# ChuckDanz/DCLIP

Measured on AMD Instinct MI355X. Metric: distill-step images/sec at ViT-B/32 bs=256, higher is better.
Workload: dtype f32

## Files before the change

dclip_amd/_lib.py:

```python
from __future__ import annotations

import ctypes as C
import os

_HERE = os.path.dirname(os.path.abspath(__file__))
LIB_PATH = os.environ.get("DCLIP_LIB_PATH") or os.path.join(_HERE, "libdclip_hip.so")

P = C.c_void_p
I = C.c_int
F = C.c_float
Z = C.c_size_t
L = C.c_int64

SIGNATURES = {
    "dclip_abi_version": (I, []),
    "dclip_last_error": (C.c_char_p, []),
    "dclip_last_launch": (C.c_char_p, []),
    "dclip_first_launch": (C.c_char_p, []),
    "dclip_gemm_f32_workspace": (Z, [I, I, I, I, I]),
    "dclip_gemm_f32_plan": (I, [I, I, I, I, I, C.POINTER(C.c_int)]),
    "dclip_gemm_f32": (I, [P, P, P, P, P, P, I, I, I, I, I, I, I, I, F, I, P, Z, P]),
    "dclip_colsum_f32_workspace": (Z, [I, I]),
    "dclip_colsum_f32": (I, [P, P, I, I, I, I, P, Z, P]),
    "dclip_layernorm_fwd": (I, [P, P, P, P, P, P, I, I, F, P]),
# ... 85 lines not shown
    "dclip_adamw_f32": (I, [P, P, P, P, Z, F, F, F, F, F, I, P, P]),
    "dclip_mt_record_bytes": (I, []),
    "dclip_mt_chunk_elems": (I, []),
    "dclip_mt_sumsq_f32": (I, [P, I, I, P, P]),
    "dclip_mt_adamw_f32": (I, [P, I, I, F, F, F, F, F, P, P]),
    "dclip_mt_adam_f32": (I, [P, I, I, F, F, F, F, F, P, P]),
    "dclip_axpby": (I, [P, P, F, F, Z, P]),
    "dclip_fill": (I, [P, F, Z, P]),
    "dclip_gemm_f16": (I, [P, P, P, P, P, I, I, I, I, I, I, I, I, P]),
    "dclip_cast_f32_f16": (I, [P, P, I, I, I, I, P]),
    "dclip_layernorm_fwd_f16": (I, [P, P, P, P, I, I, F, P]),
    "dclip_im2col_f16": (I, [P, P, I, I, I, I, I, I, P]),
    "dclip_attention_fwd_f16": (I, [P, P, I, I, I, I, P]),
    "dclip_attention_row_fwd_f16": (I, [P, P, P, I, I, I, P]),
    "dclip_split_f32_f16x3": (I, [P, P, I, I, I, I, F, I, P]),
    "dclip_layernorm_fwd_f16x3": (I, [P, P, P, P, I, I, F, F, P]),
    "dclip_gemm_f16_scaled": (I, [P, P, P, P, P, I, I, I, I, I, I, I, I, F, P]),
    "dclip_gemm_f16_scaled_split": (I, [P, P, P, P, I, I, I, I, I, I, I, F, F, P]),
    "dclip_split_f32_f16x3_dev": (I, [P, P, I, I, I, I, P, I, P]),
    "dclip_layernorm_fwd_f16x3_dev": (I, [P, P, P, P, P, P, P, I, I, F, P, P]),
    "dclip_gemm_f16_scaled_dev": (I, [P, P, P, P, P, I, I, I, I, I, I, I, I, P, P]),
    "dclip_gemm_f16_scaled_split_dev": (I, [P, P, P, P, P, P, I, I, I, I, I, I, I, P, P, P]),
    "dclip_split16_record_bytes": (I, []),
    "dclip_split16_plan_floats": (I, []),
    "dclip_split16_tile_rows": (I, []),
    "dclip_split16_stats": (I, [P, I, I, P, P]),
    "dclip_split16_plan": (I, [P, P, I, I, P]),
    "dclip_split16_weights": (I, [P, I, I, P, P]),
    "dclip_split_f32_f16x3_rows": (I, [P, P, P, I, I, I, P]),
    "dclip_split16_weights_t": (I, [P, I, I, P, P, P]),
    "dclip_gemm_f16_scaled_rows_dev": (I, [P, P, P, P, I, I, I, I, I, I, I, P, P, P]),
    "dclip_split_f32_f16x3_rows_colstats_workspace": (Z, [I, I]),
    "dclip_split_f32_f16x3_rows_colstats": (I, [P, P, P, P, P, P, P, I, I, I, P, Z, P]),
    "dclip_gemm_f16_wgrad_tokmajor_seg3_plan": (I, [I, I, I]),
    "dclip_gemm_f16_wgrad_tokmajor_seg3": (I, [P, P, P, I, I, I, I, I, I, I, I, I, I, I, I, P, P, I, P, Z, P]),
    "dclip_gemm_f16_ex": (I, [P, P, P, P, P, P, I, I, I, I, I, I, I, I, P]),
    "dclip_gemm_f16_wgrad_tokmajor_plan": (I, [I, I, I]),
    "dclip_gemm_f16_wgrad_tokmajor": (I, [P, P, P, I, I, I, I, I, I, I, P, Z, P]),
    "dclip_gemm_f16_splitk_plan": (I, [I, I, I]),
    "dclip_gemm_f16_splitk_workspace": (Z, [I, I, I]),
    "dclip_gemm_f16_splitk": (I, [P, P, P, I, I, I, I, I, I, I, P, Z, P]),
    "dclip_cast_f32_f16_ieee": (I, [P, P, I, I, I, I, P]),
    "dclip_layernorm_fwd_f16_stats": (I, [P, P, P, P, P, P, I, I, F, P]),
    "dclip_layernorm_bwd_ex_f16": (I, [P, P, P, P, P, P, P, P, P, P, P, I, I, I, P, Z, P]),
    "dclip_transpose_to_f16": (I, [P, I, P, P, I, I, I, I, I, P]),
    "dclip_rowsum_f16": (I, [P, P, I, I, I, P]),
    "dclip_colsum_f16": (I, [P, P, I, I, I, I, P, Z, P]),
    "dclip_mt_weights_f16": (I, [P, I, I, P]),
    "dclip_attention_fwd_f16_lse": (I, [P, P, P, I, I, I, I, P]),
    "dclip_attention_bwd_f16": (I, [P, P, P, P, P, I, I, I, I, P]),
    "dclip_clip_coef_scaled": (I, [P, I, F, P, P, P]),
    "dclip_mt_adamw_f32_skip": (I, [P, I, I, F, F, F, F, F, P, P]),
    "dclip_amp_update_scale": (I, [P, P, P, F, F, I, P]),
}

_lib = None


class DclipError(RuntimeError):
    pass


def load():
    global _lib
    if _lib is not None:
        return _lib
# ... 20 lines not shown
```

dclip_amd/csrc/attention.hip:

```cpp
#include "common.h"
#include "attention_tiles.h"
#include <stdlib.h>

namespace {

typedef unsigned short u16x4a __attribute__((ext_vector_type(4)));
typedef unsigned short u16x8a __attribute__((ext_vector_type(8)));
__device__ __forceinline__ f32x4 bf4_to_f32(u16x4a b) {
  f32x4 v;
#pragma unroll
  for (int e = 0; e < 4; ++e) v[e] = __builtin_bit_cast(float, (unsigned int)b[e] << 16);
  return v;
}
__device__ __forceinline__ u16x4a f32_to_bf4(f32x4 v) {
  u16x4a b;
#pragma unroll
  for (int e = 0; e < 4; ++e) b[e] = __builtin_bit_cast(unsigned short, (__bf16)v[e]);
  return b;
}
__device__ __forceinline__ void commit8(float* tile, int row, int chunk, u16x8a b, bool zero) {
  f32x4 lo, hi;
#pragma unroll
  for (int e = 0; e < 4; ++e) {
    lo[e] = zero ? 0.f : __builtin_bit_cast(float, (unsigned int)b[e] << 16);
// ... 511 lines not shown
    zero4(dpt);
    mma_rows_x_tileT(st, kf, t0, lane);
    mma_rows_x_tileT(dpt, vf, t1, lane);
#pragma unroll
    for (int nt = 0; nt < 4; ++nt) {
      const int ql = nt * 16 + l15, q = q0 + ql;
      const float lq = lse_s[ql], dq_ = dl_s[ql];
#pragma unroll
      for (int r = 0; r < 4; ++r) {
        const int key = k0 + 16 * wave + 4 * qd + r;
        const bool masked = key >= S || q >= Sq || (CAUSAL && key > q);
        const float p = masked ? 0.f : __expf(st[nt][r] * kScale - lq);
        scp[(4 * qd + r) * SCR + ql] = p;
        scs[(4 * qd + r) * SCR + ql] = p * (dpt[nt][r] - dq_) * kScale;
      }
    }
    __syncthreads();
    mma_scratch_x_tile(dv, scp, t1, lane);
    mma_scratch_x_tile(dk, scs, t0, lane);
  }
#pragma unroll
  for (int r = 0; r < 4; ++r) {
    const int key = k0 + 16 * wave + 4 * qd + r;
    if (key < S)
#pragma unroll
      for (int nt = 0; nt < 4; ++nt) {
        const size_t o = ((size_t)b * S + key) * lddkv + h * HD + nt * 16 + l15;
        dk_out[o] = dk[nt][r];
        dv_out[o] = dv[nt][r];
      }
  }
}

template <bool CAUSAL, bool IO16 = false>
__global__ void __launch_bounds__(256, 3) attn_bwd_lean_kernel(AttnArgs a, const float* __restrict__ out,
                                                               const float* __restrict__ dout, const float* __restrict__ lse,
                                                               float* __restrict__ dq_out, float* __restrict__ dk_out,
                                                               float* __restrict__ dv_out, int ldd) {
  __shared__ __attribute__((aligned(16))) float lds[3 * TS * HD + 2 * TS];
  float* Qs = lds;
  float* dOs = lds + TS * HD;
  float* dSs = lds + 2 * TS * HD;
  float* lse_s = lds + 3 * TS * HD;
  float* dl_s = lse_s + TS;
  const int H = a.H, S = a.Sk;
  const int lane = threadIdx.x & 63, wave = threadIdx.x >> 6;
  const int qd = lane >> 4, l15 = lane & 15;
  const int bh = blockIdx.x, b = bh / H, h = bh % H;
  const int D = H * HD;
  const int own = 16 * wave + l15, ownc = min(own, S - 1);
  const float my_lse = lse[(size_t)bh * S + ownc];
  f32x4 kf[4], vf[4];
  float my_dl = 0.f;
  f32x4 tk[4];
  u16x8a tk16[2];
  if constexpr (IO16) {
    const unsigned short* qb = reinterpret_cast<const unsigned short*>(a.q) + (size_t)b * S * a.ldq + h * HD;
    const unsigned short* kb = reinterpret_cast<const unsigned short*>(a.k) + (size_t)b * S * a.ldkv + h * HD;
    const unsigned short* vb = reinterpret_cast<const unsigned short*>(a.v) + (size_t)b * S * a.ldkv + h * HD;
    const unsigned short* dob = reinterpret_cast<const unsigned short*>(dout) + (size_t)b * S * D + h * HD;
    u16x8a tq16[2], tdo16[2];
    tile_fetch16(tq16, qb, S, (size_t)a.ldq);
    tile_fetch16(tdo16, dob, S, (size_t)D);
    tile_fetch16(tk16, kb, S, (size_t)a.ldkv);
    const unsigned short* krow = kb + (size_t)ownc * a.ldkv + 4 * qd;
    const unsigned short* vrow = vb + (size_t)ownc * a.ldkv + 4 * qd;
    const unsigned short* orow = reinterpret_cast<const unsigned short*>(out) + ((size_t)b * S + ownc) * D + h * HD + 4 * qd;
    const unsigned short* drow = dob + (size_t)ownc * D + 4 * qd;
#pragma unroll
    for (int g = 0; g < 4; ++g) {
      kf[g] = bf4_to_f32(*reinterpret_cast<const u16x4a*>(krow + 16 * g));
// ... 14 lines not shown
  const float* dobase = dout + (size_t)b * S * D + h * HD;
  f32x4 tq[4], tdo[4];
  tile_fetch(tq, qbase, 0, S, (size_t)a.ldq);
  tile_fetch(tdo, dobase, 0, S, (size_t)D);
  tile_fetch(tk, kbase, 0, S, (size_t)a.ldkv);
  {
    const float* krow = kbase + (size_t)ownc * a.ldkv + 4 * qd;
    const float* vrow = vbase + (size_t)ownc * a.ldkv + 4 * qd;
    const float* orow = out + ((size_t)b * S + ownc) * D + h * HD + 4 * qd;
    const float* drow = dobase + (size_t)ownc * D + 4 * qd;
#pragma unroll
    for (int g = 0; g < 4; ++g) {
      kf[g] = *reinterpret_cast<const f32x4*>(krow + 16 * g);
      vf[g] = *reinterpret_cast<const f32x4*>(vrow + 16 * g);
      const f32x4 o4 = *reinterpret_cast<const f32x4*>(orow + 16 * g);
      const f32x4 d4 = *reinterpret_cast<const f32x4*>(drow + 16 * g);
      my_dl += (o4[0] * d4[0] + o4[1] * d4[1]) + (o4[2] * d4[2] + o4[3] * d4[3]);
    }
  }
  __builtin_amdgcn_sched_barrier(0);
  tile_commit(Qs, tq, 0, S);
  tile_commit(dOs, tdo, 0, S);
#pragma unroll
  for (int c = 0; c < 4; ++c) asm volatile("" ::"v"(tk[c]));
  }
  my_dl += __shfl_xor(my_dl, 16);
  my_dl += __shfl_xor(my_dl, 32);
  if (qd == 0) {
    lse_s[own] = own < S ? my_lse : 0.f;
    dl_s[own] = own < S ? my_dl : 0.f;
  }
  __syncthreads();
  const int kts = (S + 15) / 16;
  {
    f32x4 dk[4], dv[4];
    zero4(dk);
    zero4(dv);
#pragma unroll
    for (int qt = 0; qt < 4; ++qt) {
      const bool live = qt < kts && (!CAUSAL || qt >= wave);
      f32x4 pr = {0.f, 0.f, 0.f, 0.f}, ds = {0.f, 0.f, 0.f, 0.f};
      if (live) {
        f32x4 s2 = {0.f, 0.f, 0.f, 0.f}, dp2 = {0.f, 0.f, 0.f, 0.f};
#pragma unroll
        for (int g = 0; g < 4; ++g) {
          const f32x4 qf = frag_k(Qs, 16 * qt, g, lane);
          const f32x4 df = frag_k(dOs, 16 * qt, g, lane);
#pragma unroll
          for (int r = 0; r < 4; ++r) {
            s2 = __builtin_amdgcn_mfma_f32_16x16x4f32(qf[r], kf[g][r], s2, 0, 0, 0);
            dp2 = __builtin_amdgcn_mfma_f32_16x16x4f32(df[r], vf[g][r], dp2, 0, 0, 0);
          }
        }
#pragma unroll
        for (int r = 0; r < 4; ++r) {
          const int q = 16 * qt + 4 * qd + r;
          const bool masked = q >= S || own >= S || (CAUSAL && own > q);
          pr[r] = masked ? 0.f : __expf(s2[r] * kScale - lse_s[q]);
          ds[r] = pr[r] * (dp2[r] - dl_s[q]) * kScale;
        }
#pragma unroll
        for (int r = 0; r < 4; ++r) {
          const int q = 16 * qt + 4 * qd + r;
#pragma unroll
          for (int dt = 0; dt < 4; ++dt) {
            dv[dt] = __builtin_amdgcn_mfma_f32_16x16x4f32(dOs[tile_off(q, 16 * dt + l15)], pr[r], dv[dt], 0, 0, 0);
            dk[dt] = __builtin_amdgcn_mfma_f32_16x16x4f32(Qs[tile_off(q, 16 * dt + l15)], ds[r], dk[dt], 0, 0, 0);
          }
        }
      }
#pragma unroll
      for (int r = 0; r < 4; ++r) dSs[tile_off(16 * qt + 4 * qd + r, own)] = ds[r];
    }
    if (own < S) {
      const size_t o = ((size_t)b * S + own) * ldd + h * HD + 4 * qd;
#pragma unroll
      for (int dt = 0; dt < 4; ++dt) {
        if constexpr (IO16) {
          *reinterpret_cast<u16x4a*>(reinterpret_cast<unsigned short*>(dk_out) + o + 16 * dt) = f32_to_bf4(dk[dt]);
          *reinterpret_cast<u16x4a*>(reinterpret_cast<unsigned short*>(dv_out) + o + 16 * dt) = f32_to_bf4(dv[dt]);
        } else {
          *reinterpret_cast<f32x4*>(dk_out + o + 16 * dt) = dk[dt];
          *reinterpret_cast<f32x4*>(dv_out + o + 16 * dt) = dv[dt];
        }
      }
    }
  }
  __syncthreads();
  if constexpr (IO16) tile_commit16(Qs, tk16, S);
  else tile_commit(Qs, tk, 0, S);
  __syncthreads();
  {
    const float* Ks = Qs;
    f32x4 dq[4];
    zero4(dq);
    const int n1 = CAUSAL ? min(kts, wave + 1) : kts;
#pragma unroll
    for (int kt = 0; kt < 4; ++kt)
      if (kt < n1) {
        const f32x4 dst = *reinterpret_cast<const f32x4*>(dSs + own * HD + (((4 * kt + qd) ^ (own & 15)) << 2));
#pragma unroll
        for (int r = 0; r < 4; ++r) {
          const int key = 16 * kt + 4 * qd + r;
#pragma unroll
          for (int dt = 0; dt < 4; ++dt)
            dq[dt] = __builtin_amdgcn_mfma_f32_16x16x4f32(Ks[tile_off(key, 16 * dt + l15)], dst[r], dq[dt], 0, 0, 0);
        }
      }
    if (own < S) {
      if constexpr (IO16) {
        unsigned short* o = reinterpret_cast<unsigned short*>(dq_out) + ((size_t)b * S + own) * ldd + h * HD + 4 * qd;
#pragma unroll
        for (int dt = 0; dt < 4; ++dt) *reinterpret_cast<u16x4a*>(o + 16 * dt) = f32_to_bf4(dq[dt]);
      } else {
        float* o = dq_out + ((size_t)b * S + own) * ldd + h * HD + 4 * qd;
#pragma unroll
        for (int dt = 0; dt < 4; ++dt) *reinterpret_cast<f32x4*>(o + 16 * dt) = dq[dt];
      }
    }
  }
}


template <bool CAUSAL>
__global__ void __launch_bounds__(256) attn_bwd_dq_stream_kernel(AttnArgs a, const float* __restrict__ out,
                                                                 const float* __restrict__ dout, const float* __restrict__ lse,
                                                                 float* __restrict__ dq_out, int lddq, float* __restrict__ delta) {
  __shared__ __attribute__((aligned(16))) float lds[2 * TS * HD];
  float* Ks = lds;
  float* Vs = lds + TS * HD;
  const int H = a.H, S = a.Sk;
  const int lane = threadIdx.x & 63, wave = threadIdx.x >> 6;
  const int l31 = lane & 31, half = lane >> 5;
  const int bh = blockIdx.x, b = bh / H, h = bh % H;
  const int D = H * HD;
  const int q0 = blockIdx.y * 128 + wave * 32;
  const int query = q0 + l31, qc = min(query, S - 1);
  const float* kbase = a.k + (size_t)b * S * a.ldkv + h * HD;
  const float* vbase = a.v + (size_t)b * S * a.ldkv + h * HD;
  f32x4 qf[8], dof[8];
  float my_dl = 0.f;
  {
    const float* qrow = a.q + ((size_t)b * S + qc) * a.ldq + h * HD + 4 * half;
    const float* drow = dout + ((size_t)b * S + qc) * D + h * HD + 4 * half;
    const float* orow = out + ((size_t)b * S + qc) * D + h * HD + 4 * half;
#pragma unroll
    for (int g = 0; g < 8; ++g) {
      qf[g] = *reinterpret_cast<const f32x4*>(qrow + 8 * g);
      dof[g] = *reinterpret_cast<const f32x4*>(drow + 8 * g);
      const f32x4 o4 = *reinterpret_cast<const f32x4*>(orow + 8 * g);
      my_dl += (o4[0] * dof[g][0] + o4[1] * dof[g][1]) + (o4[2] * dof[g][2] + o4[3] * dof[g][3]);
    }
  }
// ... 518 lines not shown
    return DCLIP_OK;
  }
  if (causal) {
    hipLaunchKernelGGL((attn_bwd_dq_kernel<true>), gq, block, 0, st, a, out, dout, lse, dq, lddq, delta);
    hipLaunchKernelGGL((attn_bwd_dkv_kernel<true>), gk, block, 0, st, a, dout, lse, delta, dk, dv, lddkv);
  } else {
    hipLaunchKernelGGL((attn_bwd_dq_kernel<false>), gq, block, 0, st, a, out, dout, lse, dq, lddq, delta);
    hipLaunchKernelGGL((attn_bwd_dkv_kernel<false>), gk, block, 0, st, a, dout, lse, delta, dk, dv, lddkv);
  }
  DCLIP_CHECK_LAUNCH("attention_bwd");
  return DCLIP_OK;
}

}

DCLIP_API int dclip_attention_fwd(const float* qkv, float* out, float* lse, int B, int S, int H, int causal,
                                  void* stream) {
  DCLIP_REQUIRE(qkv && out && lse, "attention_fwd: null pointer");
  DCLIP_REQUIRE(B > 0 && S > 0 && H > 0, "attention_fwd: bad shape B=%d S=%d H=%d", B, S, H);
  const int D = H * HD;
  AttnArgs a{qkv, qkv + D, qkv + 2 * D, 3 * D, 3 * D, S, S, H, nullptr};
  return launch_fwd(a, out, lse, B, causal, (hipStream_t)stream);
}

DCLIP_API int dclip_attention_bwd(const float* qkv, const float* out, const float* dout, const float* lse,
                                  float* dqkv, float* delta, int B, int S, int H, int causal, void* stream) {
  DCLIP_REQUIRE(qkv && out && dout && lse && dqkv && delta, "attention_bwd: null pointer");
  DCLIP_REQUIRE(B > 0 && S > 0 && H > 0, "attention_bwd: bad shape B=%d S=%d H=%d", B, S, H);
  const int D = H * HD;
  AttnArgs a{qkv, qkv + D, qkv + 2 * D, 3 * D, 3 * D, S, S, H, nullptr};
  return launch_bwd(a, out, dout, lse, dqkv, 3 * D, dqkv + D, dqkv + 2 * D, 3 * D, delta, B, causal, (hipStream_t)stream);
}

DCLIP_API size_t dclip_attention_bwd_workspace(int B, int S, int H, int causal) {
  size_t n = (size_t)B * H * S;
  n = (n + 63) / 64 * 64;
  if (long_noncausal(S, S, causal)) n += (size_t)B * H * ds_row_stride(S) * ds_row_stride(S);
  return n * sizeof(float);
}

DCLIP_API int dclip_attention_bwd_ws(const float* qkv, const float* out, const float* dout, const float* lse, float* dqkv,
                                     void* workspace, size_t workspace_bytes, int B, int S, int H, int causal, void* stream) {
  DCLIP_REQUIRE(qkv && out && dout && lse && dqkv && workspace, "attention_bwd_ws: null pointer");
  DCLIP_REQUIRE(B > 0 && S > 0 && H > 0, "attention_bwd_ws: bad shape B=%d S=%d H=%d", B, S, H);
  DCLIP_REQUIRE((uintptr_t)workspace % 16 == 0, "attention_bwd_ws: workspace must be 16-byte aligned");
  if (workspace_bytes < dclip_attention_bwd_workspace(B, S, H, causal)) {
    dclip_set_error("attention_bwd_ws: workspace too small (%zu < %zu)", workspace_bytes,
                    dclip_attention_bwd_workspace(B, S, H, causal));
    return DCLIP_EWORKSPACE;
  }
  const int D = H * HD;
  float* delta = (float*)workspace;
  float* ds = long_noncausal(S, S, causal) ? delta + ((size_t)B * H * S + 63) / 64 * 64 : nullptr;
  AttnArgs a{qkv, qkv + D, qkv + 2 * D, 3 * D, 3 * D, S, S, H, nullptr};
  return launch_bwd(a, out, dout, lse, dqkv, 3 * D, dqkv + D, dqkv + 2 * D, 3 * D, delta, B, causal, (hipStream_t)stream, ds);
}

DCLIP_API int dclip_attention_fwd_io16(const void* qkv16, void* out16, float* lse, int B, int S, int H, int causal, void* stream) {
  DCLIP_REQUIRE(qkv16 && out16 && lse, "attention_fwd_io16: null pointer");
  DCLIP_REQUIRE(B > 0 && S > 0 && S <= 80 && H > 0, "attention_fwd_io16: B=%d S=%d (<= 80) H=%d", B, S, H);
  DCLIP_REQUIRE(((uintptr_t)qkv16 | (uintptr_t)out16) % 16 == 0, "attention_fwd_io16: operands must be 16-byte aligned");
  const int D = H * HD;
  const float* q = reinterpret_cast<const float*>(qkv16);
  const unsigned short* q16 = reinterpret_cast<const unsigned short*>(qkv16);
  AttnArgs a{q, reinterpret_cast<const float*>(q16 + D), reinterpret_cast<const float*>(q16 + 2 * D), 3 * D, 3 * D, S, S, H, nullptr};
  hipStream_t st = (hipStream_t)stream;
// ... 92 lines not shown
```

dclip_amd/csrc/gemm_bf16.hip:

```cpp
#include "common.h"
#include <stdlib.h>
#include <type_traits>

namespace {

typedef unsigned short u16x4 __attribute__((ext_vector_type(4)));
typedef unsigned int u32x4 __attribute__((ext_vector_type(4)));
typedef unsigned int u32x2 __attribute__((ext_vector_type(2)));

constexpr int BKH = 64;

struct GemmBf16Params {
  const __bf16* A;
  const __bf16* W;
  void* C;
  const float* bias;
  const float* residual;
  int M, N, K;
  int lda, ldw, ldc;
  int epilogue;
  int out_bf16;
  int tiles_m, tiles_n;
  unsigned short* aux;
  int k_per_split;
  float* slab;
  float alpha = 1.f;
  float out_scale = 0.f;
  const float* alpha_p = nullptr;
  const float* out_scale_p = nullptr;
  float* h32 = nullptr;
  float* g32 = nullptr;
  const float* row_alpha = nullptr;
  const float* aux32 = nullptr;
  int seg_splits = 0;
  int a_seg[3] = {0, 0, 0}, w_seg[3] = {0, 0, 0};
};

__device__ __forceinline__ void store_rows4(const GemmBf16Params& p, f32x4 v, int row, size_t off) {
  v = v * p.row_alpha[row];
  if (p.epilogue & DCLIP_EPI_DGELU) {
    const f32x4 h = *reinterpret_cast<const f32x4*>(p.aux32 + off);
#pragma unroll
    for (int e = 0; e < 4; ++e) v[e] *= quick_gelu_grad_f(h[e]);
  }
  *reinterpret_cast<f32x4*>(reinterpret_cast<float*>(p.C) + off) = v;
}

__device__ __forceinline__ float dev_alpha(const GemmBf16Params& p) { return p.alpha_p ? *p.alpha_p : p.alpha; }
__device__ __forceinline__ float dev_out_scale(const GemmBf16Params& p) { return p.out_scale_p ? *p.out_scale_p : p.out_scale; }

__device__ __forceinline__ void store_split4(unsigned short* c, int N, f32x4 v, float s) {
  u16x4 hi, lo;
#pragma unroll
  for (int e = 0; e < 4; ++e) {
    float x = v[e];
    asm volatile("" : "+v"(x));
    x *= s;
    asm volatile("" : "+v"(x));
    const _Float16 h = (_Float16)x;
    const _Float16 l = (_Float16)(x - (float)h);
    hi[e] = __builtin_bit_cast(unsigned short, h);
    lo[e] = __builtin_bit_cast(unsigned short, l);
  }
  *reinterpret_cast<u16x4*>(c) = hi;
  *reinterpret_cast<u16x4*>(c + N) = lo;
  *reinterpret_cast<u16x4*>(c + 2 * N) = hi;
}

// ... 217 lines not shown
      store_split4(reinterpret_cast<unsigned short*>(p.C) + off, p.N, v, dev_out_scale(p));
    } else if (p.out_bf16) {
      u16x4 o = {T::bits(v[0]), T::bits(v[1]), T::bits(v[2]), T::bits(v[3])};
      *reinterpret_cast<u16x4*>(reinterpret_cast<unsigned short*>(p.C) + off) = o;
    } else {
      *reinterpret_cast<f32x4*>(reinterpret_cast<float*>(p.C) + off) = v;
    }
  }
}

__device__ __forceinline__ void dma16(__amdgpu_buffer_rsrc_t rsrc, __bf16* lds_dst, int voff, int soff) {
  __builtin_amdgcn_raw_ptr_buffer_load_lds(rsrc, (__attribute__((address_space(3))) void*)lds_dst, 16, voff, soff, 0, 0);
}

template <class T, int BM>
int launch_reg(const GemmBf16Params& p, size_t lds, hipStream_t st) {
  if constexpr (std::is_same<T, F16T>::value) {
    if (p.row_alpha) {
      hipLaunchKernelGGL((gemm_bf16_kernel<T, BM, BM, true>), dim3(p.tiles_m * p.tiles_n), dim3(256), lds, st, p);
      return DCLIP_OK;
    }
  }
  hipLaunchKernelGGL((gemm_bf16_kernel<T, BM, BM>), dim3(p.tiles_m * p.tiles_n), dim3(256), lds, st, p);
  return DCLIP_OK;
}

#define PP_BARRIER()                      \
  do {                                    \
    __builtin_amdgcn_sched_barrier(0);    \
    __builtin_amdgcn_s_barrier();         \
    __builtin_amdgcn_sched_barrier(0);    \
  } while (0)

template <class T, int KIND, bool OUT16, bool DEV = false, bool ROWS = false>
__device__ __forceinline__ void pp_epilogue(const GemmBf16Params& p, const f32x4 (&acc)[8][4], float* ct, int m0, int n0,
                                            int tid, int wr, int wc, int quad, int l15) {
  constexpr int BN = 256;
  const int lc = (tid & 63) * 4, col = n0 + lc, lr0 = tid >> 6;
  const bool colok = col < p.N;
  const int colc = colok ? col : 0;
  f32x4 bias4 = {0.f, 0.f, 0.f, 0.f};
  if (p.epilogue & DCLIP_EPI_BIAS) bias4 = *reinterpret_cast<const f32x4*>(p.bias + colc);
  const float alpha_d = DEV ? *p.alpha_p : 0.f;
#pragma unroll
  for (int hm = 0; hm < 2; ++hm) {
    const int rbase = m0 + hm * 128 + lr0;
    f32x4 side[KIND == 3 || (ROWS && KIND == 2) ? 16 : 1];
    u16x4 side16[KIND == 2 && !ROWS ? 16 : 1];
    if (ROWS && KIND == 2) {
#pragma unroll
      for (int q = 0; q < 16; ++q)
        side[q] = *reinterpret_cast<const f32x4*>(p.aux32 + (size_t)min(rbase + 8 * q, p.M - 1) * p.ldc + colc);
    }
    if (KIND == 3) {
#pragma unroll
      for (int q = 0; q < 16; ++q)
        side[q] = *reinterpret_cast<const f32x4*>(p.residual + (size_t)min(rbase + 8 * q, p.M - 1) * p.ldc + colc);
    }
    if (KIND == 2 && !ROWS) {
#pragma unroll
      for (int q = 0; q < 16; ++q)
        side16[q] = *reinterpret_cast<const u16x4*>(p.aux + (size_t)min(rbase + 8 * q, p.M - 1) * p.ldc + colc);
    }
    if (wr == hm) {
#pragma unroll
      for (int i = 0; i < 8; ++i)
#pragma unroll
        for (int j = 0; j < 4; ++j)
          *reinterpret_cast<f32x4*>(ct + (16 * i + l15) * BN + (((16 * wc + 4 * j + quad) ^ (l15 & 7)) << 2)) = acc[i][j];
    }
    asm volatile("s_waitcnt lgkmcnt(0)" ::: "memory");
    PP_BARRIER();
#pragma unroll
    for (int q = 0; q < 16; ++q) {
      const int row = rbase + 8 * q;
      f32x4 v = *reinterpret_cast<const f32x4*>(ct + (lr0 + 8 * q) * BN + (((tid & 63) ^ ((lr0 + 8 * q) & 7)) << 2));
      if (!ROWS) v = v * (DEV ? alpha_d : p.alpha) + bias4;
      const size_t off = (size_t)row * p.ldc + col;
      const bool ok = row < p.M && colok;
      if (ROWS) {
        if (KIND == 2) {
#pragma unroll
          for (int e = 0; e < 4; ++e) v[e] *= quick_gelu_grad_f(side[q][e]);
        }
        if (ok) *reinterpret_cast<f32x4*>(reinterpret_cast<float*>(p.C) + off) = v;
        continue;
      }
      if (KIND == 1) {
        if (DEV && !OUT16 && p.h32 && ok) *reinterpret_cast<f32x4*>(p.h32 + (size_t)row * p.N + col) = v;
        if (p.aux) {
          u16x4 h = {T::bits(v[0]), T::bits(v[1]), T::bits(v[2]), T::bits(v[3])};
          if (ok) *reinterpret_cast<u16x4*>(p.aux + off) = h;
#pragma unroll
          for (int e = 0; e < 4; ++e) v[e] = T::to_f32(h[e]);
        }
#pragma unroll
        for (int e = 0; e < 4; ++e) v[e] = quick_gelu_f(v[e]);
      }
      if (KIND == 2) {
#pragma unroll
        for (int e = 0; e < 4; ++e) v[e] *= quick_gelu_grad_f(T::to_f32(side16[q][e]));
      }
      if (KIND == 3) v += side[q];
      if (!ok) continue;
      if ((KIND == 0 || KIND == 1) && !OUT16 && p.out_scale != 0.f) {
        if (DEV && p.g32) *reinterpret_cast<f32x4*>(p.g32 + (size_t)row * p.N + col) = v;
        store_split4(reinterpret_cast<unsigned short*>(p.C) + off, p.N, v, DEV ? *p.out_scale_p : p.out_scale);
        continue;
      }
      if (OUT16) {
        u16x4 o = {T::bits(v[0]), T::bits(v[1]), T::bits(v[2]), T::bits(v[3])};
        *reinterpret_cast<u16x4*>(reinterpret_cast<unsigned short*>(p.C) + off) = o;
      } else {
        *reinterpret_cast<f32x4*>(reinterpret_cast<float*>(p.C) + off) = v;
      }
    }
    if (hm == 0) {
      asm volatile("s_waitcnt lgkmcnt(0)" ::: "memory");
      PP_BARRIER();
      PP_STAMP(3);
    }
  }
  PP_STAMP(8);
#ifdef DCLIP_GEMM_STAMPS
  asm volatile("s_waitcnt vmcnt(0)" ::: "memory");
#endif
  PP_STAMP(4);
  PP_STAMP_RT(6);
}

template <class T, bool GELU, bool SAVE, bool DEV = false>
__device__ __forceinline__ void pp_epilogue_b16(const GemmBf16Params& p, const f32x4 (&acc)[8][4], unsigned short* ct, int m0,
                                                int n0, int tid, int wr, int wc, int quad, int l15) {
  constexpr int BN = 256;
  {
    f32x4 bias4[4];
#pragma unroll
    for (int j = 0; j < 4; ++j) {
      const int col = n0 + 64 * wc + 16 * j + 4 * quad;
      bias4[j] = f32x4{0.f, 0.f, 0.f, 0.f};
      if (p.epilogue & DCLIP_EPI_BIAS) bias4[j] = *reinterpret_cast<const f32x4*>(p.bias + (col < p.N ? col : 0));
    }
    const float alpha_d = DEV ? *p.alpha_p : 0.f;
#pragma unroll
    for (int i = 0; i < 8; ++i)
#pragma unroll
      for (int j = 0; j < 4; ++j) {
        f32x4 v = acc[i][j] * (DEV ? alpha_d : p.alpha) + bias4[j];
        if (GELU && !SAVE) {
#pragma unroll
          for (int e = 0; e < 4; ++e) v[e] = quick_gelu_f(v[e]);
        }
        const u16x4 h = {T::bits(v[0]), T::bits(v[1]), T::bits(v[2]), T::bits(v[3])};
        const int row = 128 * wr + 16 * i + l15, unit = 16 * wc + 4 * j + quad;
        *reinterpret_cast<u16x4*>(ct + row * BN + ((unit ^ (row & 15)) << 2)) = h;
      }
  }
  asm volatile("s_waitcnt lgkmcnt(0)" ::: "memory");
  PP_BARRIER();
  PP_STAMP(3);
  const int cg = tid & 31, col = n0 + 8 * cg;
#pragma unroll 4
  for (int q = 0; q < 16; ++q) {
    const int lr = (tid >> 5) + 16 * q, row = m0 + lr;
    const u16x4 lo = *reinterpret_cast<const u16x4*>(ct + lr * BN + (((2 * cg) ^ (lr & 15)) << 2));
    const u16x4 hi = *reinterpret_cast<const u16x4*>(ct + lr * BN + (((2 * cg + 1) ^ (lr & 15)) << 2));
    if (row >= p.M || col >= p.N) continue;
    const size_t off = (size_t)row * p.ldc + col;
    const bool full = col + 8 <= p.N;
    typedef unsigned short u16x8 __attribute__((ext_vector_type(8)));
    u16x8 o = {lo[0], lo[1], lo[2], lo[3], hi[0], hi[1], hi[2], hi[3]};
    if (SAVE) {
      if (full) *reinterpret_cast<u16x8*>(p.aux + off) = o;
      else *reinterpret_cast<u16x4*>(p.aux + off) = lo;
#pragma unroll
      for (int e = 0; e < 8; ++e) o[e] = T::bits(quick_gelu_f(T::to_f32(o[e])));
    }
    unsigned short* c = reinterpret_cast<unsigned short*>(p.C) + off;
    if (full) *reinterpret_cast<u16x8*>(c) = o;
    else *reinterpret_cast<u16x4*>(c) = u16x4{o[0], o[1], o[2], o[3]};
  }
  PP_STAMP(8);
#ifdef DCLIP_GEMM_STAMPS
  asm volatile("s_waitcnt vmcnt(0)" ::: "memory");
#endif
  PP_STAMP(4);
  PP_STAMP_RT(6);
}

template <class T, bool TOK, bool DEV = false, bool ROWS = false, bool SEG = false>
__global__ void __launch_bounds__(512) gemm_bf16_pp_kernel(GemmBf16Params p) {
  static_assert(!SEG || (TOK && !DEV && !ROWS), "the segmented form is token-major, split-K, fp32 slabs");
  typedef typename T::x8 V8;
  constexpr int BM = 256, BN = 256, ROW = BKH;
  constexpr int BUF = (BM + BN) * ROW;
  __shared__ __attribute__((aligned(16))) unsigned char lds_raw[2 * BUF * 2];
  __bf16* lds = reinterpret_cast<__bf16*>(lds_raw);

  PP_STAMP(0);
  PP_STAMP_RT(5);
  PP_STAMP_V(7, (unsigned long long)__builtin_amdgcn_s_getreg((4) | (0 << 6) | (31 << 11)) |
                    ((unsigned long long)__builtin_amdgcn_s_getreg((20) | (0 << 6) | (3 << 11)) << 32));
  const int tid = threadIdx.x, lane = tid & 63;
  const int wave = __builtin_amdgcn_readfirstlane(tid >> 6);
  const int wr = wave >> 2, wc = wave & 3;
  const int l15 = lane & 15, quad = lane >> 4;

  constexpr int GROUP_M = 8;
  const int nwg = p.tiles_m * p.tiles_n;
  const int swz = xcd_remap16(blockIdx.x, nwg);
  const int per_group = GROUP_M * p.tiles_n;
  const int first_m = (swz / per_group) * GROUP_M;
  const int gsize = min(GROUP_M, p.tiles_m - first_m);
  const int tile_m = first_m + (swz % per_group) % gsize, tile_n = (swz % per_group) / gsize;
  const int m0 = tile_m * BM, n0 = tile_n * BN;
  int ksplit = blockIdx.y, a_col0 = 0, w_col0 = 0;
  if constexpr (SEG) {
    const int seg = (int)blockIdx.y / p.seg_splits;
    ksplit = (int)blockIdx.y - seg * p.seg_splits;
    a_col0 = seg == 0 ? p.a_seg[0] : (seg == 1 ? p.a_seg[1] : p.a_seg[2]);
    w_col0 = seg == 0 ? p.w_seg[0] : (seg == 1 ? p.w_seg[1] : p.w_seg[2]);
  }
  const int kbeg = p.k_per_split ? ksplit * p.k_per_split : 0;
  const int kspan = (p.k_per_split ? min(p.K, kbeg + p.k_per_split) : p.K) - kbeg;
  const int nk = kspan / BKH;
// ... 155 lines not shown
    __builtin_amdgcn_sched_barrier(0);
    PP_MFMA(1, 1, fb1);
    PP_BARRIER();
    if (n2) {
      if (TOK) PP_ISSUE_B(0, cur, kt + 2);
      PP_ISSUE_B(1, cur, kt + 2);
      asm volatile("s_waitcnt vmcnt(6)" ::: "memory");
    } else {
      asm volatile("s_waitcnt vmcnt(0)" ::: "memory");
    }
    PP_BARRIER();
    PP_MFMA(1, 0, fb0);
    PP_BARRIER();
  }
  if (wr == 0) PP_BARRIER();
  PP_STAMP(2);
#undef PP_ISSUE_A
#undef PP_ISSUE_B
#undef PP_READ_A
#undef PP_READ_B
#undef PP_MFMA

  const int kind = (p.epilogue & DCLIP_EPI_RESIDUAL) ? 3 : (p.epilogue & DCLIP_EPI_DGELU) ? 2 : (p.epilogue & DCLIP_EPI_GELU) ? 1 : 0;
  float* ct = reinterpret_cast<float*>(lds_raw);
  if (ROWS) {
    const float alpha_r = *p.alpha_p;
    float ra[8];
#pragma unroll
    for (int i = 0; i < 8; ++i) ra[i] = p.row_alpha[min(m0 + 128 * wr + 16 * i + l15, p.M - 1)];
#pragma unroll
    for (int i = 0; i < 8; ++i)
#pragma unroll
      for (int j = 0; j < 4; ++j) acc[i][j] = (acc[i][j] * alpha_r) * ra[i];
    if (kind == 2) pp_epilogue<T, 2, false, true, true>(p, acc, ct, m0, n0, tid, wr, wc, quad, l15);
    else pp_epilogue<T, 0, false, true, true>(p, acc, ct, m0, n0, tid, wr, wc, quad, l15);
    return;
  }
  if (!DEV && p.slab) {
    GemmBf16Params ps = p;
    ps.C = p.slab + (size_t)blockIdx.y * p.M * p.N;
    ps.ldc = p.N;
    ps.epilogue = 0;
    ps.alpha = 1.f;
    ps.out_scale = 0.f;
    pp_epilogue<T, 0, false, false>(ps, acc, ct, m0, n0, tid, wr, wc, quad, l15);
    return;
  }
  if (p.out_bf16) {
    unsigned short* ct16 = reinterpret_cast<unsigned short*>(lds_raw);
    if (kind == 0) pp_epilogue_b16<T, false, false, DEV>(p, acc, ct16, m0, n0, tid, wr, wc, quad, l15);
    else if (kind == 1 && p.aux) pp_epilogue_b16<T, true, true, DEV>(p, acc, ct16, m0, n0, tid, wr, wc, quad, l15);
    else if (kind == 1) pp_epilogue_b16<T, true, false, DEV>(p, acc, ct16, m0, n0, tid, wr, wc, quad, l15);
    else pp_epilogue<T, 2, true, DEV>(p, acc, ct, m0, n0, tid, wr, wc, quad, l15);
  } else {
    if (kind == 0) pp_epilogue<T, 0, false, DEV>(p, acc, ct, m0, n0, tid, wr, wc, quad, l15);
    else if (kind == 1) pp_epilogue<T, 1, false, DEV>(p, acc, ct, m0, n0, tid, wr, wc, quad, l15);
    else if (kind == 2) pp_epilogue<T, 2, false, DEV>(p, acc, ct, m0, n0, tid, wr, wc, quad, l15);
    else pp_epilogue<T, 3, false, DEV>(p, acc, ct, m0, n0, tid, wr, wc, quad, l15);
  }
}
#undef PP_BARRIER

#define PP_BARRIER()                      \
  do {                                    \
    __builtin_amdgcn_sched_barrier(0);    \
    __builtin_amdgcn_s_barrier();         \
    __builtin_amdgcn_sched_barrier(0);    \
  } while (0)
// ... 273 lines not shown
#pragma unroll
    for (int j = 0; j < 4; ++j) {
      const int col = pn0 + 64 * wc + 4 * quad + 16 * j;
      bias4[j] = f32x4{0.f, 0.f, 0.f, 0.f};
      if (p.epilogue & DCLIP_EPI_BIAS) bias4[j] = *reinterpret_cast<const f32x4*>(p.bias + (col < p.N ? col : 0));
    }
    store_tile(bias4);
  }
#undef PPP_ISSUE_A
#undef PPP_ISSUE_B
#undef PPP_READ_A
#undef PPP_READ_B
#undef PPP_MFMA
}
#undef PP_BARRIER

bool persistent_enabled() { return getenv("DCLIP_BF16_PERSIST") && atoi(getenv("DCLIP_BF16_PERSIST")) != 0; }

template <class T>
int launch_ppp(GemmBf16Params p, hipStream_t st) {
  p.tiles_m = cdiv(p.M, 256);
  p.tiles_n = cdiv(p.N, 256);
  const int tiles = p.tiles_m * p.tiles_n;
  int grid = tiles < 256 ? ((tiles + 7) / 8) * 8 : 256;
  hipLaunchKernelGGL(gemm_bf16_ppp_kernel<T>, dim3(grid), dim3(512), 0, st, p);
  return DCLIP_OK;
}

template <class T, bool TOK = false>
int launch_pp(GemmBf16Params p, hipStream_t st, int splits = 1) {
  p.tiles_m = cdiv(p.M, 256);
  p.tiles_n = cdiv(p.N, 256);
  if constexpr (std::is_same<T, F16T>::value && !TOK) {
    if (p.row_alpha) {
      hipLaunchKernelGGL((gemm_bf16_pp_kernel<T, false, true, true>), dim3(p.tiles_m * p.tiles_n, splits), dim3(512), 0, st, p);
      return DCLIP_OK;
    }
    if (p.alpha_p) {
      hipLaunchKernelGGL((gemm_bf16_pp_kernel<T, false, true>), dim3(p.tiles_m * p.tiles_n, splits), dim3(512), 0, st, p);
      return DCLIP_OK;
    }
  }
  hipLaunchKernelGGL((gemm_bf16_pp_kernel<T, TOK>), dim3(p.tiles_m * p.tiles_n, splits), dim3(512), 0, st, p);
  return DCLIP_OK;
}

template <class T>
__global__ void __launch_bounds__(256) cast_bf16_kernel(const float* __restrict__ x, unsigned short* __restrict__ y, int rows,
                                                        int cols, int ldx, int ldy) {
  const int ld4 = ldy >> 2;
  const size_t total = (size_t)rows * ld4;
  for (size_t i = (size_t)blockIdx.x * blockDim.x + threadIdx.x; i < total; i += (size_t)gridDim.x * blockDim.x) {
    const int c = (int)(i % ld4) * 4;
    const size_t r = i / ld4;
    u16x4 o = {0, 0, 0, 0};
    if (c + 3 < cols) {
      f32x4 v = *reinterpret_cast<const f32x4*>(x + r * ldx + c);
      o = u16x4{T::bits(v[0]), T::bits(v[1]), T::bits(v[2]), T::bits(v[3])};
    } else {
      for (int e = 0; e < 4; ++e)
        if (c + e < cols) o[e] = T::bits(x[r * ldx + c + e]);
    }
    *reinterpret_cast<u16x4*>(y + r * ldy + c) = o;
  }
}

// ... 67 lines not shown
    f32x4 s = *reinterpret_cast<const f32x4*>(slab + i * 4);
    for (int z = 1; z < splits; ++z) s += *reinterpret_cast<const f32x4*>(slab + (size_t)z * M * N + i * 4);
    const size_t row = (i * 4) / N, col = (i * 4) % N;
    *reinterpret_cast<f32x4*>(C + row * ldc + col) = (s * inv) * row_scale[row];
  }
}

inline int grid_for(size_t work) {
  size_t b = (work + 255) / 256;
  return (int)(b < 1 ? 1 : (b > 4096 ? 4096 : b));
}

}

#ifdef DCLIP_GEMM_STAMPS
DCLIP_API int dclip_debug_set_bf16_stamps(void* buf) {
  return hipMemcpyToSymbol(HIP_SYMBOL(g_stamps16), &buf, sizeof(buf)) == hipSuccess ? DCLIP_OK : DCLIP_ELAUNCH;
}
#endif

DCLIP_API int dclip_gemm_bf16(const void* A, const void* W, void* C, const float* bias, const float* residual, int M, int N,
                              int K, int lda, int ldw, int ldc, int epilogue, int out_bf16, void* stream) {
  return dclip_gemm_bf16_ex(A, W, C, bias, residual, nullptr, M, N, K, lda, ldw, ldc, epilogue, out_bf16, stream);
}

namespace {
struct DevScales {
  const float* alpha_p;
  const float* out_scale_p;
  float* h32;
  float* g32;
  const float* row_alpha = nullptr;
  const float* aux32 = nullptr;
};
inline void set_dev(GemmBf16Params& p, const DevScales* d) {
  if (d) p.alpha_p = d->alpha_p, p.out_scale_p = d->out_scale_p, p.h32 = d->h32, p.g32 = d->g32, p.row_alpha = d->row_alpha,
         p.aux32 = d->aux32;
}

template <class T>
constexpr bool kTrain16 = std::is_same<T, F16IeeeT>::value;

template <class T>
int gemm16(const char* name, const void* A, const void* W, void* C, const float* bias, const float* residual, void* aux, int M,
           int N, int K, int lda, int ldw, int ldc, int epilogue, int out_bf16, void* stream, float alpha = 1.f, float out_scale = 0.f,
           const DevScales* dev = nullptr) {
  DCLIP_REQUIRE(A && W && C, "%s: null operand", name);
  DCLIP_REQUIRE(M > 0 && N > 0 && K > 0, "%s: bad shape M=%d N=%d K=%d", name, M, N, K);
  DCLIP_REQUIRE(lda % 8 == 0 && ldw % 8 == 0 && lda >= K && ldw >= K, "%s: lda/ldw must be multiples of 8 and >= K", name);
  DCLIP_REQUIRE(N % 4 == 0 && ldc % 4 == 0 && ldc >= N, "%s: N / ldc must be multiples of 4", name);
  DCLIP_REQUIRE(((uintptr_t)A | (uintptr_t)W | (uintptr_t)C) % 16 == 0, "%s: operands must be 16-byte aligned", name);
  DCLIP_REQUIRE(!(epilogue & ~(DCLIP_EPI_BIAS | DCLIP_EPI_GELU | DCLIP_EPI_DGELU | DCLIP_EPI_RESIDUAL)),
                "%s: unsupported epilogue bits", name);
  DCLIP_REQUIRE(out_scale == 0.f || (!out_bf16 && !aux && !(epilogue & (DCLIP_EPI_RESIDUAL | DCLIP_EPI_DGELU)) && (long)ldc >= 3L * N),
                "%s: a split output takes BIAS | GELU only and ldc >= 3 N", name);
  DCLIP_REQUIRE(!(epilogue & DCLIP_EPI_DGELU) || ((aux || (dev && dev->aux32)) && !(epilogue & DCLIP_EPI_GELU)),
                "%s: DGELU needs aux (and no GELU)", name);
  DCLIP_REQUIRE(!aux || (uintptr_t)aux % 8 == 0, "%s: aux must be 8-byte aligned", name);
  DCLIP_REQUIRE(!(epilogue & DCLIP_EPI_BIAS) || bias, "%s: BIAS without bias", name);
  DCLIP_REQUIRE(!(epilogue & DCLIP_EPI_RESIDUAL) || (residual && !out_bf16), "%s: RESIDUAL needs an fp32 output", name);
  hipStream_t st = (hipStream_t)stream;
  const int big_min = getenv("DCLIP_BF16_BIG_MIN") ? atoi(getenv("DCLIP_BF16_BIG_MIN")) : 128;
  if (K % BKH == 0 && (long)cdiv(M, 256) * cdiv(N, 256) >= big_min) {
    GemmBf16Params pb{(const __bf16*)A, (const __bf16*)W, C, bias, residual, M, N, K, lda, ldw, ldc, epilogue, out_bf16, 0, 0,
                      (unsigned short*)aux, 0, nullptr, alpha, out_scale};
    set_dev(pb, dev);
    if constexpr (!kTrain16<T>) {
      const int persist_min = getenv("DCLIP_BF16_PERSIST_MIN") ? atoi(getenv("DCLIP_BF16_PERSIST_MIN")) : 512;
      const bool gelu_f32 = (epilogue & DCLIP_EPI_GELU) && !out_bf16;
      if (persistent_enabled() && !(epilogue & DCLIP_EPI_DGELU) && !gelu_f32 && out_scale == 0.f && !dev && ldc % 8 == 0 &&
          N % 8 == 0 && (long)cdiv(M, 256) * cdiv(N, 256) >= persist_min) {
        launch_ppp<T>(pb, st);
        DCLIP_CHECK_LAUNCH_V(name, ".ppp");
        return DCLIP_OK;
      }
    }
    launch_pp<T>(pb, st);
    DCLIP_CHECK_LAUNCH_V(name, ".pp");
    return DCLIP_OK;
  }
  const bool small = (long)cdiv(M, 128) * cdiv(N, 128) < 256;
  const int bm = small ? 64 : 128, bn = bm;
  GemmBf16Params p{(const __bf16*)A, (const __bf16*)W, C, bias, residual, M, N, K, lda, ldw, ldc, epilogue, out_bf16,
                   cdiv(M, bm), cdiv(N, bn), (unsigned short*)aux, 0, nullptr, alpha, out_scale};
  set_dev(p, dev);
  const size_t lds = (size_t)2 * (bm + bn) * BKH * 2;
  if (small) launch_reg<T, 64>(p, lds, st);
  else launch_reg<T, 128>(p, lds, st);
  DCLIP_CHECK_LAUNCH_V(name, small ? ".r64" : ".r128");
  return DCLIP_OK;
}
}

DCLIP_API int dclip_gemm_bf16_ex(const void* A, const void* W, void* C, const float* bias, const float* residual, void* aux,
                                 int M, int N, int K, int lda, int ldw, int ldc, int epilogue, int out_bf16, void* stream) {
  return gemm16<Bf16T>("gemm_bf16", A, W, C, bias, residual, aux, M, N, K, lda, ldw, ldc, epilogue, out_bf16, stream);
// ... 30 lines not shown
  const DevScales dev{alpha, nullptr, nullptr, nullptr};
  return gemm16<F16T>("gemm_f16_scaled_dev", A, W, C, bias, residual, nullptr, M, N, K, lda, ldw, ldc, epilogue, out_f16, stream, 1.f,
                      0.f, &dev);
}

DCLIP_API int dclip_gemm_f16_scaled_split_dev(const void* A, const void* W, void* C, const float* bias, float* h32, float* g32, int M,
                                              int N, int K, int lda, int ldw, int ldc, int epilogue, const float* alpha,
                                              const float* out_scale, void* stream) {
  DCLIP_REQUIRE(alpha && ((uintptr_t)alpha | (uintptr_t)out_scale) % 4 == 0,
                "gemm_f16_scaled_split_dev: alpha / out_scale must be device pointers");
  DCLIP_REQUIRE(ldc % 8 == 0, "gemm_f16_scaled_split_dev: ldc must be a multiple of 8");
  DCLIP_REQUIRE(((uintptr_t)h32 | (uintptr_t)g32) % 16 == 0, "gemm_f16_scaled_split_dev: h32 / g32 must be 16-byte aligned");
  DCLIP_REQUIRE(!h32 || (epilogue & DCLIP_EPI_GELU), "gemm_f16_scaled_split_dev: h32 is the pre-activation of a GELU epilogue");
  DCLIP_REQUIRE(!(epilogue & ~(DCLIP_EPI_BIAS | DCLIP_EPI_GELU)), "gemm_f16_scaled_split_dev: the epilogue is BIAS | GELU");
  DCLIP_REQUIRE(out_scale || !g32, "gemm_f16_scaled_split_dev: without out_scale C is the fp32 result (g32 must be NULL)");
  const DevScales dev{alpha, out_scale, h32, g32};
  return gemm16<F16T>("gemm_f16_scaled_split_dev", A, W, C, bias, nullptr, nullptr, M, N, K, lda, ldw, ldc, epilogue, 0, stream, 1.f,
                      out_scale ? 1.f : 0.f, &dev);
}

DCLIP_API int dclip_gemm_f16_scaled_rows_dev(const void* A, const void* W, float* C, const float* aux32, int M, int N, int K, int lda,
                                             int ldw, int ldc, int epilogue, const float* alpha, const float* row_alpha,
                                             void* stream) {
  DCLIP_REQUIRE(alpha && row_alpha && ((uintptr_t)alpha | (uintptr_t)row_alpha) % 4 == 0,
                "gemm_f16_scaled_rows_dev: alpha / row_alpha must be device pointers");
  DCLIP_REQUIRE(epilogue == 0 || epilogue == DCLIP_EPI_DGELU, "gemm_f16_scaled_rows_dev: the epilogue is none or DGELU");
  DCLIP_REQUIRE(!(epilogue & DCLIP_EPI_DGELU) || (aux32 && (uintptr_t)aux32 % 16 == 0),
                "gemm_f16_scaled_rows_dev: DGELU needs a 16-byte aligned fp32 aux32");
  DevScales dev{alpha, nullptr, nullptr, nullptr};
  dev.row_alpha = row_alpha;
  dev.aux32 = (epilogue & DCLIP_EPI_DGELU) ? aux32 : nullptr;
  return gemm16<F16T>("gemm_f16_scaled_rows_dev", A, W, C, nullptr, nullptr, nullptr, M, N, K, lda, ldw, ldc, epilogue, 0, stream, 1.f,
                      0.f, &dev);
}

DCLIP_API int dclip_gemm_f16_ex(const void* A, const void* W, void* C, const float* bias, const float* residual, void* aux,
                                int M, int N, int K, int lda, int ldw, int ldc, int epilogue, int out_f16, void* stream) {
  return gemm16<F16IeeeT>("gemm_f16_ex", A, W, C, bias, residual, aux, M, N, K, lda, ldw, ldc, epilogue, out_f16, stream);
}

namespace {
int tokmajor_plan(int M, int N, int K) {
  if (K % BKH != 0 || M % 8 != 0 || N % 8 != 0) return 0;
  const long t256 = (long)cdiv(M, 256) * cdiv(N, 256);
  int s = t256 >= 256 ? 1 : (int)(256 / t256);
  const int kmax = K / 512 > 0 ? K / 512 : 1;
  s = s > kmax ? kmax : s;
  s = s > 64 ? 64 : s;
  return t256 * s >= 128 ? s : 0;
}

template <class T>
int wgrad_tokmajor16(const char* name, const void* dY, const void* X, float* C, int M, int N, int K, int lddy, int ldx, int ldc,
                     int splits, void* workspace, size_t workspace_bytes, void* stream) {
  DCLIP_REQUIRE(dY && X && C, "%s: null operand", name);
  DCLIP_REQUIRE(M > 0 && N > 0 && K > 0 && K % BKH == 0 && M % 8 == 0 && N % 8 == 0 && splits >= 1 && splits <= 64,
                "%s: M=%d N=%d (multiples of 8) K=%d (multiple of 64) splits=%d", name, M, N, K, splits);
  DCLIP_REQUIRE(lddy % 8 == 0 && ldx % 8 == 0 && lddy >= M && ldx >= N && ldc % 4 == 0 && ldc >= N, "%s: leading dimensions", name);
  DCLIP_REQUIRE(((uintptr_t)dY | (uintptr_t)X | (uintptr_t)C) % 16 == 0, "%s: operands must be 16-byte aligned", name);
  const int kps = cdiv(cdiv(K, splits), BKH) * BKH;
  const int s_eff = cdiv(K, kps);
  hipStream_t st = (hipStream_t)stream;
  if (s_eff == 1) {
    GemmBf16Params pb{(const __bf16*)dY, (const __bf16*)X, C, nullptr, nullptr, M, N, K, lddy, ldx, ldc, 0, 0, 0, 0, nullptr, 0, nullptr};
    launch_pp<T, true>(pb, st, 1);
    DCLIP_CHECK_LAUNCH_V(name, ".pp_tok");
// ... 238 lines not shown
```

dclip_amd/csrc/layernorm.hip:

```cpp
#include "common.h"

namespace {

constexpr int MAXC = 8;

template <int NC, bool EXACT>
__global__ void __launch_bounds__(256) ln_fwd_kernel(const float* __restrict__ x, const float* __restrict__ gamma,
                                                     const float* __restrict__ beta, float* __restrict__ y,
                                                     float* __restrict__ mean, float* __restrict__ rstd, int rows,
                                                     int D, float eps) {
  const int lane = threadIdx.x & 63;
  const int row = blockIdx.x * 4 + (threadIdx.x >> 6);
  if (row >= rows) return;
  const int d4 = D >> 2;
  const f32x4* xr = reinterpret_cast<const f32x4*>(x + (size_t)row * D);
  f32x4 v[NC], g[NC], bt[NC];
#pragma unroll
  for (int c = 0; c < NC; ++c) {
    const int i = lane + 64 * c, ic = (EXACT || i < d4) ? i : 0;
    v[c] = xr[ic];
    g[c] = reinterpret_cast<const f32x4*>(gamma)[ic];
    bt[c] = reinterpret_cast<const f32x4*>(beta)[ic];
  }
  float s = 0.f;
#pragma unroll
  for (int c = 0; c < NC; ++c) {
    if (!EXACT && lane + 64 * c >= d4) v[c] = f32x4{0.f, 0.f, 0.f, 0.f};
    s += (v[c][0] + v[c][1]) + (v[c][2] + v[c][3]);
  }
  const float mu = wave_sum(s) / (float)D;
  float q = 0.f;
#pragma unroll
  for (int c = 0; c < NC; ++c) {
    if (EXACT || lane + 64 * c < d4) {
      f32x4 d = v[c] - mu;
      q += (d[0] * d[0] + d[1] * d[1]) + (d[2] * d[2] + d[3] * d[3]);
    }
  }
  const float rs = rsqrtf(wave_sum(q) / (float)D + eps);
  if (lane == 0) {
    if (mean) mean[row] = mu;
    if (rstd) rstd[row] = rs;
  }
  f32x4* yr = reinterpret_cast<f32x4*>(y + (size_t)row * D);
#pragma unroll
  for (int c = 0; c < NC; ++c) {
    const int i = lane + 64 * c;
    if (EXACT || i < d4) yr[i] = (v[c] - mu) * rs * g[c] + bt[c];
  }
}

template <class T, int NC, bool EXACT>
__global__ void __launch_bounds__(256) ln_bwd_kernel(const float* __restrict__ dy, const float* __restrict__ x,
                                                     const float* __restrict__ gamma, const float* __restrict__ mean,
                                                     const float* __restrict__ rstd, const float* __restrict__ dres,
                                                     float* __restrict__ dx, float* __restrict__ partial, int rows,
                                                     int D, unsigned short* __restrict__ dx16, int NS) {
  extern __shared__ __attribute__((aligned(16))) float red[];
  const int lane = threadIdx.x & 63, wave = threadIdx.x >> 6;
  const int d4 = D >> 2;
  f32x4 g[NC], dg[NC], db[NC], dsum[NC];
#pragma unroll
  for (int c = 0; c < NC; ++c) {
    int i = lane + 64 * c;
    g[c] = (EXACT || i < d4) ? reinterpret_cast<const f32x4*>(gamma)[i] : f32x4{0.f, 0.f, 0.f, 0.f};
    dg[c] = f32x4{0.f, 0.f, 0.f, 0.f};
    db[c] = f32x4{0.f, 0.f, 0.f, 0.f};
    dsum[c] = f32x4{0.f, 0.f, 0.f, 0.f};
  }
  const float invD = 1.0f / (float)D;
  const bool has_res = dres != nullptr;
  for (int row = blockIdx.x * 4 + wave; row < rows; row += gridDim.x * 4) {
    const f32x4* xr = reinterpret_cast<const f32x4*>(x + (size_t)row * D);
    const f32x4* dyr = reinterpret_cast<const f32x4*>(dy + (size_t)row * D);
    const f32x4* rr = reinterpret_cast<const f32x4*>((has_res ? dres : dy) + (size_t)row * D);
    const float mu = mean[row], rs = rstd[row];
    f32x4 xh[NC], dyh[NC], rv[NC];
#pragma unroll
    for (int c = 0; c < NC; ++c) {
      const int i = lane + 64 * c, ic = (EXACT || i < d4) ? i : 0;
      dyh[c] = dyr[ic];
      xh[c] = xr[ic];
      rv[c] = rr[ic];
    }
    float s1 = 0.f, s2 = 0.f;
#pragma unroll
    for (int c = 0; c < NC; ++c) {
      if (EXACT || lane + 64 * c < d4) {
        const f32x4 dyv = dyh[c];
        xh[c] = (xh[c] - mu) * rs;
        dg[c] += dyv * xh[c];
        db[c] += dyv;
        dyh[c] = dyv * g[c];
        f32x4 t = dyh[c] * xh[c];
        s1 += (t[0] + t[1]) + (t[2] + t[3]);
        s2 += (dyh[c][0] + dyh[c][1]) + (dyh[c][2] + dyh[c][3]);
      } else {
        xh[c] = f32x4{0.f, 0.f, 0.f, 0.f};
        dyh[c] = f32x4{0.f, 0.f, 0.f, 0.f};
      }
    }
    const float c1 = wave_sum(s1) * invD, c2 = wave_sum(s2) * invD;
    f32x4* dxr = reinterpret_cast<f32x4*>(dx + (size_t)row * D);
#pragma unroll
    for (int c = 0; c < NC; ++c) {
      const int i = lane + 64 * c;
      if (EXACT || i < d4) {
        f32x4 o = (dyh[c] - c2 - xh[c] * c1) * rs;
        if (has_res) o += rv[c];
        dxr[i] = o;
        if (NS == 3) dsum[c] += o;
        if (dx16) {
          typedef unsigned short u16x4_t __attribute__((ext_vector_type(4)));
          u16x4_t b;
#pragma unroll
          for (int e = 0; e < 4; ++e) b[e] = T::bits(o[e]);
          *reinterpret_cast<u16x4_t*>(dx16 + (size_t)row * D + i * 4) = b;
        }
      }
    }
  }
  if (partial) {
#pragma unroll
    for (int c = 0; c < NC; ++c) {
      int i = lane + 64 * c;
      if (EXACT || i < d4) {
        reinterpret_cast<f32x4*>(red + (wave * NS + 0) * D)[i] = dg[c];
        reinterpret_cast<f32x4*>(red + (wave * NS + 1) * D)[i] = db[c];
        if (NS == 3) reinterpret_cast<f32x4*>(red + (wave * NS + 2) * D)[i] = dsum[c];
      }
    }
    __syncthreads();
    const int W = NS * D;
    for (int i = threadIdx.x; i < W; i += 256) {
      float s = red[i] + red[W + i] + red[2 * W + i] + red[3 * W + i];
      partial[(size_t)blockIdx.x * W + i] = s;
    }
  }
}

constexpr int RP_COLS = 16, RP_GROUPS = 64;
__global__ void __launch_bounds__(1024) reduce_partials_kernel(const float* __restrict__ partial, float* __restrict__ out0,
                                                               float* __restrict__ out1, int P, int N0, int N1,
                                                               int accumulate, float* __restrict__ out2 = nullptr, int N2 = 0) {
  __shared__ float red[RP_GROUPS][RP_COLS + 1];
  __shared__ float red2[4][RP_COLS];
  const int cl = threadIdx.x % RP_COLS, rg = threadIdx.x / RP_COLS;
  const int n = blockIdx.x * RP_COLS + cl;
  const int N = N0 + N1 + N2;
  float s = 0.f;
  if (n < N)
    for (int p = rg; p < P; p += RP_GROUPS) s += partial[(size_t)p * N + n];
  red[rg][cl] = s;
  __syncthreads();
  if (threadIdx.x < RP_COLS * 4) {
    const int c = threadIdx.x % RP_COLS, q = threadIdx.x / RP_COLS;
    float t = 0.f;
#pragma unroll
    for (int k = 0; k < 16; ++k) t += red[q * 16 + k][c];
    red2[q][c] = t;
  }
  __syncthreads();
  if (threadIdx.x >= RP_COLS || n >= N) return;
  s = (red2[0][cl] + red2[1][cl]) + (red2[2][cl] + red2[3][cl]);
  float* base = (n < N0) ? out0 : (n < N0 + N1 ? out1 : out2);
  if (!base) return;
  float* o = base + ((n < N0) ? n : (n < N0 + N1 ? n - N0 : n - N0 - N1));
  *o = (accumulate && n < N0 + N1) ? *o + s : s;
}

template <class T>
// ... 154 lines not shown
  DCLIP_REQUIRE((uintptr_t)X % 8 == 0, "%s: alignment", name);
  const int splits = colsum_splits(M);
  if (!workspace || workspace_bytes < (size_t)splits * N * sizeof(float)) {
    dclip_set_error("%s: workspace too small", name);
    return DCLIP_EWORKSPACE;
  }
  hipStream_t st = (hipStream_t)stream;
  hipLaunchKernelGGL(colsum_bf16_kernel<T>, dim3(cdiv(N / 4, 64), splits), dim3(256), 0, st, (const unsigned short*)X,
                     (float*)workspace, M, N, ldx);
  DCLIP_CHECK_LAUNCH(name);
  hipLaunchKernelGGL(reduce_partials_kernel, dim3(cdiv(N, RP_COLS)), dim3(1024), 0, st, (const float*)workspace, out,
                     (float*)nullptr, splits, N, 0, accumulate);
  DCLIP_CHECK_LAUNCH(name);
  return DCLIP_OK;
}
}

DCLIP_API int dclip_layernorm_bwd_ex(const float* dy, const float* x, const float* gamma, const float* mean,
                                     const float* rstd, const float* dresidual, float* dx, void* dx_bf16, float* dgamma,
                                     float* dbeta, float* dx_colsum, int rows, int D, int accumulate_param_grads,
                                     void* workspace, size_t workspace_bytes, void* stream) {
  return layernorm_bwd16<Bf16T>("layernorm_bwd", dy, x, gamma, mean, rstd, dresidual, dx, dx_bf16, dgamma, dbeta, dx_colsum,
                                rows, D, accumulate_param_grads, workspace, workspace_bytes, stream);
}

DCLIP_API int dclip_layernorm_bwd_ex_f16(const float* dy, const float* x, const float* gamma, const float* mean,
                                         const float* rstd, const float* dresidual, float* dx, void* dx_f16, float* dgamma,
                                         float* dbeta, float* dx_colsum, int rows, int D, int accumulate_param_grads,
                                         void* workspace, size_t workspace_bytes, void* stream) {
  return layernorm_bwd16<F16IeeeT>("layernorm_bwd_f16", dy, x, gamma, mean, rstd, dresidual, dx, dx_f16, dgamma, dbeta, dx_colsum,
                                   rows, D, accumulate_param_grads, workspace, workspace_bytes, stream);
}

DCLIP_API size_t dclip_colsum_f32_workspace(int M, int N) { return (size_t)colsum_splits(M) * N * sizeof(float); }

DCLIP_API int dclip_colsum_f32(const float* X, float* out, int M, int N, int ldx, int accumulate, void* workspace,
                               size_t workspace_bytes, void* stream) {
  DCLIP_REQUIRE(X && out, "colsum: null pointer");
  DCLIP_REQUIRE(M > 0 && N > 0 && N % 4 == 0 && ldx % 4 == 0 && ldx >= N, "colsum: bad shape M=%d N=%d ldx=%d", M, N, ldx);
  const int splits = colsum_splits(M);
  if (!workspace || workspace_bytes < (size_t)splits * N * sizeof(float)) {
    dclip_set_error("colsum: workspace too small");
    return DCLIP_EWORKSPACE;
  }
  hipStream_t st = (hipStream_t)stream;
  hipLaunchKernelGGL(colsum_kernel, dim3(cdiv(N / 4, 64), splits), dim3(256), 0, st, X, (float*)workspace, M, N, ldx);
  DCLIP_CHECK_LAUNCH("colsum");
  hipLaunchKernelGGL(reduce_partials_kernel, dim3(cdiv(N, RP_COLS)), dim3(1024), 0, st, (const float*)workspace, out,
                     (float*)nullptr, splits, N, 0, accumulate);
  DCLIP_CHECK_LAUNCH("colsum.reduce");
  return DCLIP_OK;
}

DCLIP_API int dclip_colsum_bf16(const void* X, float* out, int M, int N, int ldx, int accumulate, void* workspace,
                                size_t workspace_bytes, void* stream) {
  return colsum16<Bf16T>("colsum_bf16", X, out, M, N, ldx, accumulate, workspace, workspace_bytes, stream);
}

DCLIP_API int dclip_colsum_f16(const void* X, float* out, int M, int N, int ldx, int accumulate, void* workspace,
                               size_t workspace_bytes, void* stream) {
  return colsum16<F16IeeeT>("colsum_f16", X, out, M, N, ldx, accumulate, workspace, workspace_bytes, stream);
}
```

dclip_amd/csrc/split16.hip:

```cpp
#include "common.h"

namespace {

typedef unsigned short u16x4 __attribute__((ext_vector_type(4)));
typedef unsigned short u16x8 __attribute__((ext_vector_type(8)));
typedef unsigned int u32x4s __attribute__((ext_vector_type(4)));
typedef int i32x4s __attribute__((ext_vector_type(4)));

__device__ __forceinline__ void split1(float v, unsigned short& hi, unsigned short& lo) {
  asm volatile("" : "+v"(v));
  const _Float16 h = (_Float16)v;
  const _Float16 l = (_Float16)(v - (float)h);
  hi = __builtin_bit_cast(unsigned short, h);
  lo = __builtin_bit_cast(unsigned short, l);
}

template <int ORDER>
__global__ void __launch_bounds__(256) split_f16x3_kernel(const float* __restrict__ x, unsigned short* __restrict__ y, int rows,
                                                          int cols, int ldx, int ldy, float scale_v,
                                                          const float* __restrict__ scale_p) {
  const float scale = scale_p ? *scale_p : scale_v;
  const int c8 = cols >> 3;
  const size_t total = (size_t)rows * c8;
  for (size_t i = (size_t)blockIdx.x * blockDim.x + threadIdx.x; i < total; i += (size_t)gridDim.x * blockDim.x) {
// ... 227 lines not shown
  if (g == 0 && col < cols) {
    for (int k = 1; k < FIN_GROUPS; ++k) {
      m = m > smax[k][cl] ? m : smax[k][cl];
      s += ssum[k][cl];
    }
    const int e = row_exp(m);
    col_exp[col] = e;
    col_alpha[col] = pow2f(-e);
    if (db) db[col] = s;
  }
}

__global__ void __launch_bounds__(256) split_cols_f16x2_kernel(const float* __restrict__ x, const int* __restrict__ col_exp,
                                                               unsigned short* __restrict__ yc, int rows, int cols, int ldx) {
  const int c8 = cols >> 3;
  const size_t total = (size_t)rows * c8;
  for (size_t i = (size_t)blockIdx.x * blockDim.x + threadIdx.x; i < total; i += (size_t)gridDim.x * blockDim.x) {
    const int c = (int)(i % c8) * 8;
    const size_t r = i / c8;
    const f32x4 a = *reinterpret_cast<const f32x4*>(x + r * ldx + c);
    const f32x4 b = *reinterpret_cast<const f32x4*>(x + r * ldx + c + 4);
    const i32x4s ea = *reinterpret_cast<const i32x4s*>(col_exp + c), eb = *reinterpret_cast<const i32x4s*>(col_exp + c + 4);
    u16x8 hi, lo;
#pragma unroll
    for (int e = 0; e < 4; ++e) {
      unsigned short h0, l0, h1, l1;
      split1(a[e] * pow2f(ea[e]), h0, l0);
      split1(b[e] * pow2f(eb[e]), h1, l1);
      hi[e] = h0, lo[e] = l0, hi[4 + e] = h1, lo[4 + e] = l1;
    }
    unsigned short* yr = yc + r * 2 * cols + c;
    *reinterpret_cast<u16x8*>(yr) = hi;
    *reinterpret_cast<u16x8*>(yr + cols) = lo;
  }
}

template <int NC, bool EXACT>
__global__ void __launch_bounds__(256) ln_fwd_f16x3_kernel(const float* __restrict__ x, const float* __restrict__ gamma,
                                                           const float* __restrict__ beta, unsigned short* __restrict__ y,
                                                           int rows, int D, float eps, float scale_v,
                                                           const float* __restrict__ scale_p, float* __restrict__ y32,
                                                           float* __restrict__ mean, float* __restrict__ rstd) {
  const float scale = scale_p ? *scale_p : scale_v;
  const int lane = threadIdx.x & 63;
  const int row = blockIdx.x * 4 + (threadIdx.x >> 6);
  if (row >= rows) return;
  const int d4 = D >> 2;
  const f32x4* xr = reinterpret_cast<const f32x4*>(x + (size_t)row * D);
  f32x4 v[NC], g[NC], bt[NC];
#pragma unroll
  for (int c = 0; c < NC; ++c) {
    const int i = lane + 64 * c, ic = (EXACT || i < d4) ? i : 0;
    v[c] = xr[ic];
    g[c] = reinterpret_cast<const f32x4*>(gamma)[ic];
    bt[c] = reinterpret_cast<const f32x4*>(beta)[ic];
  }
  float s = 0.f;
#pragma unroll
  for (int c = 0; c < NC; ++c) {
    if (!EXACT && lane + 64 * c >= d4) v[c] = f32x4{0.f, 0.f, 0.f, 0.f};
    s += (v[c][0] + v[c][1]) + (v[c][2] + v[c][3]);
  }
  const float mu = wave_sum(s) / (float)D;
  float q = 0.f;
#pragma unroll
  for (int c = 0; c < NC; ++c) {
// ... 269 lines not shown
  else if (nc == 6) SPLITROWS(6);
  else SPLITROWS(0);
#undef SPLITROWS
  DCLIP_CHECK_LAUNCH_V("split_f32_f16x3_rows", variant);
  return DCLIP_OK;
}

int split_rows_colstats_launch(const float* x, void* y, float* row_alpha, unsigned* pmax, float* psum, int rows, int cols, int ldx,
                                void* stream) {
  dim3 grid(colstat_waves(rows) / 4), block(256);
  hipStream_t st = (hipStream_t)stream;
  unsigned short* yy = (unsigned short*)y;
  const int nc = cdiv(cols / 8, 64);
  const char* variant;
#define SPLITROWSC(NC)                                                                                                        \
  do {                                                                                                                        \
    hipLaunchKernelGGL((split_rows_colstats_f16x3_kernel<NC>), grid, block, 0, st, x, yy, row_alpha, pmax, psum, rows, cols,  \
                       ldx);                                                                                                  \
    variant = (NC) ? ".regs.nc" #NC : ".cached";                                                                              \
  } while (0)
  if (nc <= 1) SPLITROWSC(1);
  else if (nc == 2) SPLITROWSC(2);
  else if (nc == 3) SPLITROWSC(3);
  else if (nc == 4) SPLITROWSC(4);
  else if (nc == 5) SPLITROWSC(5);
  else if (nc == 6) SPLITROWSC(6);
  else SPLITROWSC(0);
#undef SPLITROWSC
  DCLIP_CHECK_LAUNCH_V("split_f32_f16x3_rows_colstats", variant);
  dclip_note_first_launch("split_f32_f16x3_rows_colstats", variant);
  return DCLIP_OK;
}

int ln_launch(const char* name, const float* x, const float* gamma, const float* beta, void* y, int rows, int D, float eps,
              float scale, const float* scale_p, float* y32, float* mean, float* rstd, void* stream) {
  dim3 grid(cdiv(rows, 4)), block(256);
  hipStream_t st = (hipStream_t)stream;
  const int nc = cdiv(D / 4, 64);
  unsigned short* yy = (unsigned short*)y;
  const char* variant;
#define LN16X3(NC, EX)                                                                                                      \
  do {                                                                                                                      \
    hipLaunchKernelGGL((ln_fwd_f16x3_kernel<NC, EX>), grid, block, 0, st, x, gamma, beta, yy, rows, D, eps, scale, scale_p, \
                       y32, mean, rstd);                                                                                    \
    variant = (EX) ? ".nc" #NC ".exact" : ".nc" #NC;                                                                        \
  } while (0)
  if (D == 512) LN16X3(2, true);
  else if (D == 768) LN16X3(3, true);
  else if (D == 1024) LN16X3(4, true);
  else if (nc <= 1) LN16X3(1, false);
  else if (nc == 2) LN16X3(2, false);
  else if (nc == 3) LN16X3(3, false);
  else if (nc == 4) LN16X3(4, false);
  else LN16X3(8, false);
#undef LN16X3
  DCLIP_CHECK_LAUNCH_V(name, variant);
  return DCLIP_OK;
}

}

DCLIP_API int dclip_split_f32_f16x3(const float* x, void* y, int rows, int cols, int ldx, int ldy, float scale, int order,
                                    void* stream) {
  DCLIP_REQUIRE(x && y && rows > 0 && cols > 0, "split_f32_f16x3: bad arguments");
  DCLIP_REQUIRE(cols % 8 == 0, "split_f32_f16x3: cols=%d must be a multiple of 8", cols);
  DCLIP_REQUIRE(ldx >= cols && ldx % 4 == 0 && ldy % 8 == 0 && (long)ldy >= 3L * cols,
// ... 29 lines not shown
}

DCLIP_API int dclip_split_f32_f16x3_rows_colstats(const float* x, void* y, float* row_alpha, void* yc, int* col_exp, float* col_alpha,
                                                  float* db, int rows, int cols, int ldx, void* workspace, size_t workspace_bytes,
                                                  void* stream) {
  dclip_note_first_launch("", "");
  DCLIP_REQUIRE(x && y && row_alpha && yc && col_exp && col_alpha && rows > 0 && cols > 0, "split_f32_f16x3_rows_colstats: bad arguments");
  DCLIP_REQUIRE(cols % 8 == 0, "split_f32_f16x3_rows_colstats: cols=%d must be a multiple of 8", cols);
  DCLIP_REQUIRE(ldx >= cols && ldx % 4 == 0, "split_f32_f16x3_rows_colstats: ldx must be a multiple of 4 and >= cols");
  DCLIP_REQUIRE(((uintptr_t)x | (uintptr_t)y | (uintptr_t)yc | (uintptr_t)col_exp | (uintptr_t)workspace) % 16 == 0 &&
                    ((uintptr_t)row_alpha | (uintptr_t)col_alpha | (uintptr_t)db) % 4 == 0,
                "split_f32_f16x3_rows_colstats: alignment");
  const size_t need = dclip_split_f32_f16x3_rows_colstats_workspace(rows, cols);
  if (!workspace || workspace_bytes < need) {
    dclip_set_error("split_f32_f16x3_rows_colstats: needs %zu workspace bytes, got %zu", need, workspace_bytes);
    return DCLIP_EWORKSPACE;
  }
  const int W = colstat_waves(rows);
  unsigned* pmax = (unsigned*)workspace;
  float* psum = (float*)workspace + (size_t)W * cols;
  const int rc = split_rows_colstats_launch(x, y, row_alpha, pmax, psum, rows, cols, ldx, stream);
  if (rc != DCLIP_OK) return rc;
  hipStream_t st = (hipStream_t)stream;
  hipLaunchKernelGGL(colstats_finish_kernel, dim3(cdiv(cols, FIN_COLS)), dim3(256), 0, st, (const unsigned*)pmax, (const float*)psum, col_exp,
                     col_alpha, db, W < rows ? W : rows, cols);
  DCLIP_CHECK_LAUNCH_V("split_f32_f16x3_rows_colstats", ".finish");
  const size_t blocks = ((size_t)rows * (cols / 8) + 255) / 256;
  hipLaunchKernelGGL(split_cols_f16x2_kernel, dim3((unsigned)(blocks > 8192 ? 8192 : blocks)), dim3(256), 0, st, x, (const int*)col_exp,
                     (unsigned short*)yc, rows, cols, ldx);
  DCLIP_CHECK_LAUNCH_V("split_f32_f16x3_rows_colstats", ".cols");
  return DCLIP_OK;
}

DCLIP_API int dclip_layernorm_fwd_f16x3(const float* x, const float* gamma, const float* beta, void* y, int rows, int D,
                                        float eps, float scale, void* stream) {
  DCLIP_REQUIRE(x && gamma && beta && y, "layernorm_fwd_f16x3: null pointer");
  DCLIP_REQUIRE(rows > 0 && D > 0 && D % 4 == 0 && D <= 2048, "layernorm_fwd_f16x3: bad D=%d", D);
  DCLIP_REQUIRE(((uintptr_t)x | (uintptr_t)gamma | (uintptr_t)beta) % 16 == 0 && (uintptr_t)y % 8 == 0,
                "layernorm_fwd_f16x3: alignment");
  DCLIP_REQUIRE(pow2(scale), "layernorm_fwd_f16x3: scale must be a power of two");
  return ln_launch("layernorm_fwd_f16x3", x, gamma, beta, y, rows, D, eps, scale, nullptr, nullptr, nullptr, nullptr, stream);
}

DCLIP_API int dclip_layernorm_fwd_f16x3_dev(const float* x, const float* gamma, const float* beta, void* y, float* y32, float* mean,
                                            float* rstd, int rows, int D, float eps, const float* scale, void* stream) {
  DCLIP_REQUIRE(x && gamma && beta && y && scale, "layernorm_fwd_f16x3_dev: null pointer");
  DCLIP_REQUIRE(rows > 0 && D > 0 && D % 4 == 0 && D <= 2048, "layernorm_fwd_f16x3_dev: bad D=%d", D);
  DCLIP_REQUIRE(((uintptr_t)x | (uintptr_t)gamma | (uintptr_t)beta | (uintptr_t)y32) % 16 == 0 && (uintptr_t)y % 8 == 0 &&
                    (uintptr_t)scale % 4 == 0,
                "layernorm_fwd_f16x3_dev: alignment");
  return ln_launch("layernorm_fwd_f16x3_dev", x, gamma, beta, y, rows, D, eps, 1.f, scale, y32, mean, rstd, stream);
}

DCLIP_API int dclip_split16_record_bytes(void) { return (int)sizeof(Split16Ref); }
DCLIP_API int dclip_split16_plan_floats(void) { return PLAN_FLOATS; }
DCLIP_API int dclip_split16_tile_rows(void) { return SPLIT16_TILE_ROWS; }

DCLIP_API int dclip_split16_stats(const void* refs, int nrefs, int tiles, void* stats, void* stream) {
  DCLIP_REQUIRE(refs && stats && nrefs > 0 && tiles > 0, "split16_stats: bad arguments");
  hipLaunchKernelGGL(split16_stats_kernel, dim3(tiles), dim3(256), 0, (hipStream_t)stream, (const Split16Ref*)refs, nrefs,
                     (unsigned*)stats);
  DCLIP_CHECK_LAUNCH("split16_stats");
  return DCLIP_OK;
}

DCLIP_API int dclip_split16_plan(void* stats, float* plan, int nlayers, int D, void* stream) {
// ... 22 lines not shown
```

dclip_amd/engine.py:

```python
from __future__ import annotations

from dataclasses import dataclass
from typing import Dict, List, Optional

import os

import torch

from . import _lib, ops


@dataclass
class LayerParams:
    ln1_w: torch.Tensor
    ln1_b: torch.Tensor
    qkv_w: torch.Tensor
    qkv_b: torch.Tensor
    out_w: torch.Tensor
    out_b: torch.Tensor
    ln2_w: torch.Tensor
    ln2_b: torch.Tensor
    fc1_w: torch.Tensor
    fc1_b: torch.Tensor
    fc2_w: torch.Tensor
# ... 48 lines not shown
        return g3, h, g
    g = ops.gemm_f16_dev(a, sp.w["fc1"], sp.alpha("fc1"), bias=p.fc1_b, gelu=True, h32=h)
    return ops.split_f16x3_dev(g, sp.act("g")), h, g


def layer_fwd(x, p: LayerParams, B: int, S: int, H: int, causal: bool, eps: float, save: bool, sp: Optional[Split16Layer] = None,
              keep_split: bool = False):
    a1, ln1, m1, r1 = _ln_operand(x, p.ln1_w, p.ln1_b, eps, save, sp, "ln1")
    qkv = _linear(a1, p.qkv_w, sp, "qkv", p.qkv_b)
    attn, lse = ops.attention_fwd(qkv, B, S, H, causal)
    ac = attn if sp is None else ops.split_f16x3_dev(attn, sp.act("ctx"))
    x1 = _linear(ac, p.out_w, sp, "out", p.out_b, residual=x)
    a2, ln2, m2, r2 = _ln_operand(x1, p.ln2_w, p.ln2_b, eps, save, sp, "ln2")
    ag, h, g = _fc1_gelu(a2, p, save, sp)
    x2 = _linear(ag, p.fc2_w, sp, "fc2", p.fc2_b, residual=x1)
    saved = (x, m1, r1, ln1, qkv, attn, lse, x1, m2, r2, ln2, h, g) if save else None
    if save and keep_split and sp is not None:
        saved = saved + ({"ln1": a1, "ctx": ac, "ln2": a2, "g": ag},)
    return x2, saved


def _fresh(_name: str, shape, device) -> torch.Tensor:
    return torch.empty(shape, dtype=torch.float32, device=device)


def _galloc(alloc, name: str, shape, device) -> torch.Tensor:
    t = alloc(name, shape) if alloc is not None else None
    return t if t is not None else _fresh(name, shape, device)


def linear_param_grads(dy, x, need_w: bool, need_b: bool, gr: Dict[str, torch.Tensor], wkey: str, bkey: str, alloc=None,
                       sp: Optional[Split16Layer] = None, act: Optional[str] = None, x3: Optional[torch.Tensor] = None):
    dev = dy.device
    if (need_w and sp is not None and x3 is not None and _VSPLIT16_WGRAD and dy.dim() == 2 and dy.stride(1) == 1 and
            ops.gemm_f16_wgrad_tokmajor_seg3_plan(dy.shape[1], x.shape[1], dy.shape[0]) > 0):
        M, N = dy.shape[1], x.shape[1]
        db = _galloc(alloc, bkey, (M,), dev) if need_b else None
        dy3, row_alpha, yc, _, col_alpha = ops.split_f16x3_rows_colstats(dy, db=db)
        if need_b:
            gr[bkey] = db
        gr[wkey] = ops.gemm_f16_wgrad_tokmajor_seg3(yc, x3, M, N, col_alpha, sp.act(act), out=_galloc(alloc, wkey, (M, N), dev))
        return dy3, row_alpha
    if need_w and need_b:
        gr[bkey] = _galloc(alloc, bkey, (dy.shape[1],), dev)
        gr[wkey] = ops.gemm(dy, x, ops.LAYOUT_TN, out=_galloc(alloc, wkey, (dy.shape[1], x.shape[1]), dev), a_rowsum=gr[bkey])
    elif need_w:
        gr[wkey] = ops.gemm(dy, x, ops.LAYOUT_TN, out=_galloc(alloc, wkey, (dy.shape[1], x.shape[1]), dev))
    elif need_b:
        gr[bkey] = ops.colsum(dy, out=_galloc(alloc, bkey, (dy.shape[1],), dev))
    return None


def _ln_bwd(dy, x, gamma, mean, rstd, dresidual, want: bool, gr, wkey: str, bkey: str, alloc):
    if want:
        dg = _galloc(alloc, wkey, tuple(gamma.shape), dy.device)
        db = _galloc(alloc, bkey, tuple(gamma.shape), dy.device)
        dx, dg, db = ops.layernorm_bwd(dy, x, gamma, mean, rstd, dresidual=dresidual, dgamma=dg, dbeta=db, accumulate=False)
        gr[wkey], gr[bkey] = dg, db
        return dx
    dx, _, _ = ops.layernorm_bwd(dy, x, gamma, mean, rstd, dresidual=dresidual, need_param_grads=False)
    return dx


def _dgrad(dy, w, sp: Optional[Split16Layer], name: str, aux=None, rows=None):
    if sp is None:
        if aux is None:
            return ops.gemm(dy, w, ops.LAYOUT_NN)
        return ops.gemm(dy, w, ops.LAYOUT_NN, aux=aux, epilogue=ops.EPI_DGELU)
    dy3, row_alpha = rows if rows is not None else ops.split_f16x3_rows(dy)
    return ops.gemm_f16_rows_dev(dy3, sp.wt[name], sp.walpha(name), row_alpha, dgelu_h=aux)


def layer_bwd(dx2, p: LayerParams, saved, B: int, S: int, H: int, causal: bool, need: Dict[str, bool], alloc=None,
              sp: Optional[Split16Layer] = None):
    x, m1, r1, ln1, qkv, attn, lse, x1, m2, r2, ln2, h, g = saved[:13]
    s3 = saved[13] if len(saved) > 13 and sp is not None else {}
    gr: Dict[str, torch.Tensor] = {}
    rows = linear_param_grads(dx2, g, bool(need.get("fc2_w")), bool(need.get("fc2_b")), gr, "fc2_w", "fc2_b", alloc, sp, "g", s3.get("g"))
    dh = _dgrad(dx2, p.fc2_w, sp, "fc2", aux=h, rows=rows)
    rows = linear_param_grads(dh, ln2, bool(need.get("fc1_w")), bool(need.get("fc1_b")), gr, "fc1_w", "fc1_b", alloc, sp, "ln2",
                              s3.get("ln2"))
    dln2 = _dgrad(dh, p.fc1_w, sp, "fc1", rows=rows)
    del dh
    dx1 = _ln_bwd(dln2, x1, p.ln2_w, m2, r2, dx2, bool(need.get("ln2_w") or need.get("ln2_b")), gr, "ln2_w", "ln2_b", alloc)
    rows = linear_param_grads(dx1, attn, bool(need.get("out_w")), bool(need.get("out_b")), gr, "out_w", "out_b", alloc, sp, "ctx",
                              s3.get("ctx"))
    dattn = _dgrad(dx1, p.out_w, sp, "out", rows=rows)
    dqkv = ops.attention_bwd(qkv, attn, dattn, lse, B, S, H, causal)
    rows = linear_param_grads(dqkv, ln1, bool(need.get("qkv_w")), bool(need.get("qkv_b")), gr, "qkv_w", "qkv_b", alloc, sp, "ln1",
                              s3.get("ln1"))
    dln1 = _dgrad(dqkv, p.qkv_w, sp, "qkv", rows=rows)
    del dqkv, rows
    dx = _ln_bwd(dln1, x, p.ln1_w, m1, r1, dx1, bool(need.get("ln1_w") or need.get("ln1_b")), gr, "ln1_w", "ln1_b", alloc)
    return dx, gr



def last_layer_fwd_cls(x, p: LayerParams, B: int, S: int, H: int, eps: float, save: bool, sp: Optional[Split16Layer] = None,
                       keep_split: bool = False):
    D = x.shape[1]
    a, ln1, m1, r1 = _ln_operand(x, p.ln1_w, p.ln1_b, eps, save, sp, "ln1")
    qkv = _linear(a, p.qkv_w, sp, "qkv", p.qkv_b)
    attn, lse = ops.attention_cls_fwd(qkv, B, S, H)
    x_cls = ops.gather_rows(x, None, B, S, D)
    x1 = ops.gemm(attn, p.out_w, ops.LAYOUT_NT, bias=p.out_b, residual=x_cls)
    ln2, m2, r2 = ops.layernorm_fwd(x1, p.ln2_w, p.ln2_b, eps, save_stats=save)
    h = torch.empty((B, p.fc1_w.shape[0]), dtype=torch.float32, device=x.device) if save else None
    g = ops.gemm(ln2, p.fc1_w, ops.LAYOUT_NT, bias=p.fc1_b, aux=h, epilogue=ops.EPI_GELU)
    x2 = ops.gemm(g, p.fc2_w, ops.LAYOUT_NT, bias=p.fc2_b, residual=x1)
    saved = (x, m1, r1, ln1, qkv, attn, lse, x1, m2, r2, ln2, h, g) if save else None
    if save and keep_split and sp is not None:
        saved = saved + ({"ln1": a},)
    return x2, saved


def last_layer_bwd_cls(dx2, p: LayerParams, saved, B: int, S: int, H: int, need: Dict[str, bool], alloc=None,
                       sp: Optional[Split16Layer] = None):
    x, m1, r1, ln1, qkv, attn, lse, x1, m2, r2, ln2, h, g = saved[:13]
    s3 = saved[13] if len(saved) > 13 and sp is not None else {}
    D = x.shape[1]
    gr: Dict[str, torch.Tensor] = {}
    linear_param_grads(dx2, g, bool(need.get("fc2_w")), bool(need.get("fc2_b")), gr, "fc2_w", "fc2_b", alloc)
    dh = ops.gemm(dx2, p.fc2_w, ops.LAYOUT_NN, aux=h, epilogue=ops.EPI_DGELU)
    linear_param_grads(dh, ln2, bool(need.get("fc1_w")), bool(need.get("fc1_b")), gr, "fc1_w", "fc1_b", alloc)
    dln2 = ops.gemm(dh, p.fc1_w, ops.LAYOUT_NN)
    dx1 = _ln_bwd(dln2, x1, p.ln2_w, m2, r2, dx2, bool(need.get("ln2_w") or need.get("ln2_b")), gr, "ln2_w", "ln2_b", alloc)
    linear_param_grads(dx1, attn, bool(need.get("out_w")), bool(need.get("out_b")), gr, "out_w", "out_b", alloc)
    dattn = ops.gemm(dx1, p.out_w, ops.LAYOUT_NN)
    dqkv = ops.attention_cls_bwd(qkv, attn, dattn, lse, B, S, H)
    rows = linear_param_grads(dqkv, ln1, bool(need.get("qkv_w")), bool(need.get("qkv_b")), gr, "qkv_w", "qkv_b", alloc, sp, "ln1",
                              s3.get("ln1"))
    dln1 = _dgrad(dqkv, p.qkv_w, sp, "qkv", rows=rows)
    del dqkv, rows
    dres = ops.scatter_rows(dx1, None, B, S, D)
    dx = _ln_bwd(dln1, x, p.ln1_w, m1, r1, dres, bool(need.get("ln1_w") or need.get("ln1_b")), gr, "ln1_w", "ln1_b", alloc)
    return dx, gr



@dataclass
class VisionParams:
    class_embedding: torch.Tensor
    patch_w: torch.Tensor
    pos: torch.Tensor
    pre_w: torch.Tensor
    pre_b: torch.Tensor
    layers: List[LayerParams]
    post_w: torch.Tensor
    post_b: torch.Tensor
    proj_w: torch.Tensor

    HEAD = ("class_embedding", "patch_w", "pos", "pre_w", "pre_b")
    TAIL = ("post_w", "post_b", "proj_w")

    def tensors(self):
        out = [getattr(self, f) for f in self.HEAD]
        for l in self.layers:
            out += l.tensors()
        out += [getattr(self, f) for f in self.TAIL]
        return out

    @classmethod
    def from_tensors(cls, ts, n_layers):
        ts = list(ts)
        head = ts[:5]
        layers = [LayerParams(*ts[5 + 12 * i: 5 + 12 * (i + 1)]) for i in range(n_layers)]
        tail = ts[5 + 12 * n_layers:]
        return cls(*head, layers, *tail)
# ... 59 lines not shown
        cls_tok = ops.gather_rows(x, None, B, S, D)
    pooled, mp, rp = ops.layernorm_fwd(cls_tok, p.post_w, p.post_b, v.layer_norm_eps, save_stats=save)
    out = ops.gemm(pooled, p.proj_w, ops.LAYOUT_NT)
    saved = (cols, emb, m0, r0, saved_layers, cls_tok, mp, rp, pooled, prune, grid) if save else None
    return out, saved


def vision_bwd(p: VisionParams, saved, d_out: torch.Tensor, cfg, need: List[bool], on_ready=None, alloc=None, split16=None):
    v = cfg
    cols, emb, m0, r0, saved_layers, cls_tok, mp, rp, pooled, pruned, grid = saved
    B = cls_tok.shape[0]
    S, D, H = _grid_seq(v, grid), v.hidden_size, v.num_attention_heads
    names = p.names()
    needd = dict(zip(names, need))
    grads: Dict[str, Optional[torch.Tensor]] = {n: None for n in names}
    dev = d_out.device
    if needd["proj_w"]:
        grads["proj_w"] = ops.gemm(d_out, pooled, ops.LAYOUT_TN, out=_galloc(alloc, "proj_w", tuple(p.proj_w.shape), dev))
    dpooled = ops.gemm(d_out, p.proj_w, ops.LAYOUT_NN)
    dcls = _ln_bwd(dpooled, cls_tok, p.post_w, mp, rp, None, bool(needd["post_w"] or needd["post_b"]), grads, "post_w", "post_b",
                   alloc)
    if on_ready is not None:
        on_ready({n: grads[n] for n in VisionParams.TAIL if grads[n] is not None})
    n_layers = len(p.layers)
    lowest = None
    for i, n in enumerate(names):
        if needd[n] and n not in VisionParams.TAIL:
            li = -1 if n in VisionParams.HEAD else int(n.split(".")[1])
            lowest = li if lowest is None else min(lowest, li)
    if lowest is None:
        return [grads[n] for n in names]
    dx = None if pruned else ops.scatter_rows(dcls, None, B, S, D)
    plan = split16.layers if split16 is not None and _VSPLIT16_BWD and split16.fresh() else None
    for i in range(n_layers - 1, max(lowest, 0) - 1, -1):
        lneed = {f: needd[f"layers.{i}.{f}"] for f in LayerParams.FIELDS}
        lalloc = None if alloc is None else (lambda f, shape, i=i: alloc(f"layers.{i}.{f}", shape))
        sp = plan[i] if plan is not None else None
        if pruned and i == n_layers - 1:
            dx, gr = last_layer_bwd_cls(dcls, p.layers[i], saved_layers[i], B, S, H, lneed, lalloc, sp)
        else:
            dx, gr = layer_bwd(dx, p.layers[i], saved_layers[i], B, S, H, False, lneed, lalloc, sp)
        saved_layers[i] = None
        for f, t in gr.items():
            grads[f"layers.{i}.{f}"] = t
        if on_ready is not None:
            on_ready({f"layers.{i}.{f}": t for f, t in gr.items()})
    if lowest < 0:
        demb = _ln_bwd(dx, emb, p.pre_w, m0, r0, None, bool(needd["pre_w"] or needd["pre_b"]), grads, "pre_w", "pre_b", alloc)
        if needd["pos"] or needd["class_embedding"]:
            dpos = ops.colsum(demb.view(B, S * D),
                              out=(_galloc(alloc, "pos", (S * D,), dev) if needd["pos"] and grid is None else None))
            if needd["pos"]:
                grads["pos"] = dpos.view(S, D) if grid is None else _grid_pos_grad(dpos, p, v, grid, alloc, dev)
            if needd["class_embedding"]:
                ce = _galloc(alloc, "class_embedding", (D,), dev)
                ce.copy_(dpos[:D])
                grads["class_embedding"] = ce
        if needd["patch_w"]:
            dpatch = ops.vision_assemble_bwd(demb, B, S, D)
            pw = _galloc(alloc, "patch_w", (D, p.patch_w.numel() // D), dev)
            grads["patch_w"] = ops.gemm(dpatch, cols, ops.LAYOUT_TN, out=pw).view_as(p.patch_w)
        if on_ready is not None:
            on_ready({n: grads[n] for n in VisionParams.HEAD if grads[n] is not None})
    return [grads[n] for n in names]




class _Ops16:

    def __init__(self, dtype, gemm, layernorm, attention, attention_row, cast, im2col, im2col_rect, attention_varlen,
                 attention_varlen_row):
        self.dtype, self._gemm, self.layernorm, self.attention = dtype, gemm, layernorm, attention
        self.attention_row, self.cast, self.im2col, self.im2col_rect = attention_row, cast, im2col, im2col_rect
# ... 701 lines not shown
    B, T = input_ids.shape
    H, eps = t.num_attention_heads, t.layer_norm_eps
    eos = ops.first_eos(input_ids, t.eos_token_id)
    x = ops.text_embed_fwd(input_ids, p.tok, p.pos)
    for lp, ent in zip(p.layers[:-1], plan[:-1]):
        e = ent["e"]
        ln1 = ops.layernorm_fwd_f16x3(x, lp.ln1_w, lp.ln1_b, eps, 2.0 ** e["ln1"])
        qkv = _split16_gemm(ln1, ent, "qkv", "ln1", bias=lp.qkv_b)
        attn, _ = ops.attention_fwd(qkv, B, T, H, True)
        x1 = _split16_gemm(ops.split_f16x3(attn, 2.0 ** e["ctx"]), ent, "out", "ctx", bias=lp.out_b, residual=x)
        ln2 = ops.layernorm_fwd_f16x3(x1, lp.ln2_w, lp.ln2_b, eps, 2.0 ** e["ln2"])
        if _SPLIT16_FC1_EPI:
            g3 = _split16_gemm(ln2, ent, "fc1", "ln2", bias=lp.fc1_b, gelu=True, split_out_scale=2.0 ** e["g"])
        else:
            g3 = ops.split_f16x3(_split16_gemm(ln2, ent, "fc1", "ln2", bias=lp.fc1_b, gelu=True), 2.0 ** e["g"])
        x = _split16_gemm(g3, ent, "fc2", "g", bias=lp.fc2_b, residual=x1)
    lp, ent = p.layers[-1], plan[-1]
    ln1 = ops.layernorm_fwd_f16x3(x, lp.ln1_w, lp.ln1_b, eps, 2.0 ** ent["e"]["ln1"])
    qkv = _split16_gemm(ln1, ent, "qkv", "ln1", bias=lp.qkv_b)
    attn = ops.attention_row_fwd(qkv, eos, B, T, H)
    x1 = ops.gemm(attn, lp.out_w, ops.LAYOUT_NT, bias=lp.out_b, residual=ops.gather_rows(x, eos, B, T, D))
    ln2, _, _ = ops.layernorm_fwd(x1, lp.ln2_w, lp.ln2_b, eps, save_stats=False)
    g = ops.gemm(ln2, lp.fc1_w, ops.LAYOUT_NT, bias=lp.fc1_b, epilogue=ops.EPI_GELU)
    rows = ops.gemm(g, lp.fc2_w, ops.LAYOUT_NT, bias=lp.fc2_b, residual=x1)
    pooled, _, _ = ops.layernorm_fwd(rows, p.final_w, p.final_b, eps, save_stats=False)
    return ops.gemm(pooled, p.proj_w, ops.LAYOUT_NT)



_VSPLIT16 = os.environ.get("DCLIP_VISION_SPLIT16", "1") != "0"
_VSPLIT16_FC1_EPI = os.environ.get("DCLIP_VISION_SPLIT16_FC1_EPI", "1") != "0"
_VSPLIT16_BWD = os.environ.get("DCLIP_VISION_SPLIT16_BWD", "1") != "0"
_VSPLIT16_WGRAD = os.environ.get("DCLIP_VISION_SPLIT16_WGRAD", "1") != "0"


def vision_split16_enabled() -> bool:
    return _VSPLIT16


def split16_plan_host(st: Dict[str, float], D: int) -> Dict[str, object]:
    import math
    flags = 0
    e, f = {}, {}
    for k, b in split16_layer_bounds(st, D).items():
        x = split16_act_exp(b)
        if x is None:
            if not math.isfinite(b) or b < 0.0:
                flags |= 2
                x = 0
            else:
                flags |= 1
                m, ex = math.frexp(b)
                x = _SPLIT16_TOP - (ex - 1 if m == 0.5 else ex)
        e[k] = x
    for short, _ in _TRAIN_WEIGHTS:
        if math.isfinite(st[short]):
            f[short] = split16_weight_exp(st[short])
        else:
            flags |= 2
            f[short] = 0
    a = {}
    for short, akey in (("qkv", "ln1"), ("out", "ctx"), ("fc1", "ln2"), ("fc2", "g")):
        if e[akey] < -126:
            e[akey], flags = -126, flags | 4
        if f[short] > 127:
            f[short], flags = 127, flags | 4
# ... 320 lines not shown
```

dclip_amd/ops.py:

```python
from __future__ import annotations

from typing import Optional

import torch

from . import _lib

A_KMAJOR, B_KMAJOR = 1, 2
EPI_BIAS, EPI_GELU, EPI_DGELU, EPI_RESIDUAL, EPI_ACCUM, EPI_A_ROWSUM = 1, 2, 4, 8, 16, 32
LAYOUT_NT = A_KMAJOR | B_KMAJOR
LAYOUT_NN = A_KMAJOR
LAYOUT_TN = 0


def _stream():
    return torch.cuda.current_stream().cuda_stream


def _f32(t: torch.Tensor, name: str) -> torch.Tensor:
    if not (t.is_cuda and t.dtype == torch.float32 and t.is_contiguous()):
        raise ValueError(f"{name}: expected a contiguous float32 CUDA tensor, got {t.dtype} {t.device} "
                         f"contiguous={t.is_contiguous()}")
    return t

# ... 13 lines not shown
            return None
        key = device.index
        b = self.buf.get(key)
        if b is None or b.numel() < nbytes:
            if torch.cuda.is_current_stream_capturing():
                raise RuntimeError("workspace growth inside a HIP-graph capture: run the step eagerly once before "
                                   "capturing (GraphedStep does)")
            if b is not None:
                self.retired.append(b)
            b = torch.empty(max(nbytes, 2 * (b.numel() if b is not None else 0), 1 << 20), dtype=torch.uint8, device=device)
            self.buf[key] = b
        return b


_ws = _Workspace()
_ws_lanes = {0: _ws}


class workspace_lane:

    def __init__(self, lane: int):
        self.lane = lane

    def __enter__(self):
        global _ws
        self.prev = _ws
        _ws = _ws_lanes.setdefault(self.lane, _Workspace())
        return self

    def __exit__(self, *exc):
        global _ws
        _ws = self.prev
        return False



def gemm(a: torch.Tensor, b: torch.Tensor, layout: int, *, out: Optional[torch.Tensor] = None,
         bias: Optional[torch.Tensor] = None, residual: Optional[torch.Tensor] = None,
         aux: Optional[torch.Tensor] = None, epilogue: int = 0, alpha: float = 1.0, split_k: int = 0,
         a_rowsum: Optional[torch.Tensor] = None) -> torch.Tensor:
    lib = _lib.load()
    _f32(a, "a"), _f32(b, "b")
    if a.dim() != 2 or b.dim() != 2:
        raise ValueError("gemm: 2-D operands")
    if layout & A_KMAJOR:
        M, K = a.shape
    else:
        K, M = a.shape
    if layout & B_KMAJOR:
        N, Kb = b.shape
    else:
        Kb, N = b.shape
    if K != Kb:
        raise ValueError(f"gemm: contraction mismatch {tuple(a.shape)} x {tuple(b.shape)} layout={layout}")
    if out is None:
        out = torch.empty((M, N), dtype=torch.float32, device=a.device)
    _f32(out, "out")
    if tuple(out.shape) != (M, N):
        raise ValueError(f"gemm: out shape {tuple(out.shape)} != {(M, N)}")
    if bias is not None:
        epilogue |= EPI_BIAS
        if _f32(bias, "bias").numel() != N:
            raise ValueError("gemm: bias size")
    if residual is not None:
        epilogue |= EPI_RESIDUAL
        if tuple(_f32(residual, "residual").shape) != (M, N):
# ... 18 lines not shown
    _f32(x, "x")
    M, N = x.shape
    if out is None:
        out = torch.empty((N,), dtype=torch.float32, device=x.device)
        accumulate = False
    _f32(out, "out")
    if out.numel() != N:
        raise ValueError("colsum: out size")
    nbytes = lib.dclip_colsum_f32_workspace(M, N)
    ws = _ws.get(nbytes, x.device)
    _lib.check(lib.dclip_colsum_f32(x.data_ptr(), out.data_ptr(), M, N, N, int(accumulate), _ptr(ws), nbytes,
                                    _stream()), "colsum")
    return out



def layernorm_fwd(x: torch.Tensor, gamma: torch.Tensor, beta: torch.Tensor, eps: float, save_stats: bool = True):
    lib = _lib.load()
    _f32(x, "x"), _f32(gamma, "gamma"), _f32(beta, "beta")
    D = x.shape[-1]
    rows = x.numel() // D
    if gamma.numel() != D or beta.numel() != D:
        raise ValueError("layernorm: gamma/beta size")
    y = torch.empty_like(x)
    mean = torch.empty((rows,), dtype=torch.float32, device=x.device) if save_stats else None
    rstd = torch.empty((rows,), dtype=torch.float32, device=x.device) if save_stats else None
    _lib.check(lib.dclip_layernorm_fwd(x.data_ptr(), gamma.data_ptr(), beta.data_ptr(), y.data_ptr(), _ptr(mean),
                                       _ptr(rstd), rows, D, float(eps), _stream()), "layernorm_fwd")
    return y, mean, rstd


def layernorm_bwd(dy, x, gamma, mean, rstd, *, dresidual=None, dgamma=None, dbeta=None, accumulate=False,
                  need_param_grads=True, want_bf16: bool = False, dx_colsum: Optional[torch.Tensor] = None,
                  dtype16: torch.dtype = torch.bfloat16):
    lib = _lib.load()
    _f32(dy, "dy"), _f32(x, "x"), _f32(gamma, "gamma"), _f32(mean, "mean"), _f32(rstd, "rstd")
    D = x.shape[-1]
    rows = x.numel() // D
    if dy.shape != x.shape or mean.numel() != rows or rstd.numel() != rows or gamma.numel() != D:
        raise ValueError("layernorm_bwd: shape mismatch")
    if dresidual is not None and _f32(dresidual, "dresidual").shape != x.shape:
        raise ValueError("layernorm_bwd: dresidual shape")
    dx = torch.empty_like(x)
    if need_param_grads:
        if dgamma is None:
            dgamma = torch.empty_like(gamma)
            dbeta = torch.empty_like(gamma)
            accumulate = False
        _f32(dgamma, "dgamma"), _f32(dbeta, "dbeta")
        if dgamma.numel() != D or dbeta.numel() != D:
            raise ValueError("layernorm_bwd: dgamma/dbeta size")
    else:
        dgamma = dbeta = None
    if dx_colsum is not None and (_f32(dx_colsum, "dx_colsum").numel() != D):
        raise ValueError("layernorm_bwd: dx_colsum size")
    nbytes = lib.dclip_layernorm_bwd_workspace(rows, D) if (need_param_grads or dx_colsum is not None) else 0
    ws = _ws.get(nbytes, x.device)
    if not want_bf16 and dx_colsum is None:
        _lib.check(lib.dclip_layernorm_bwd(dy.data_ptr(), x.data_ptr(), gamma.data_ptr(), mean.data_ptr(),
                                           rstd.data_ptr(), _ptr(dresidual), dx.data_ptr(), _ptr(dgamma), _ptr(dbeta),
                                           rows, D, int(accumulate), _ptr(ws), nbytes, _stream()), "layernorm_bwd")
        return dx, dgamma, dbeta
    if dtype16 not in (torch.bfloat16, torch.float16):
        raise ValueError(f"layernorm_bwd: dtype16 {dtype16}")
    dx16 = torch.empty(x.shape, dtype=dtype16, device=x.device) if want_bf16 else None
    entry = lib.dclip_layernorm_bwd_ex if dtype16 == torch.bfloat16 else lib.dclip_layernorm_bwd_ex_f16
    _lib.check(entry(dy.data_ptr(), x.data_ptr(), gamma.data_ptr(), mean.data_ptr(), rstd.data_ptr(),
                                          _ptr(dresidual), dx.data_ptr(), _ptr(dx16), _ptr(dgamma), _ptr(dbeta),
                                          _ptr(dx_colsum), rows, D, int(accumulate), _ptr(ws), nbytes, _stream()),
               "layernorm_bwd_ex")
    return (dx, dgamma, dbeta, dx16) if want_bf16 else (dx, dgamma, dbeta)



def attention_fwd(qkv: torch.Tensor, B: int, S: int, H: int, causal: bool):
    lib = _lib.load()
    _f32(qkv, "qkv")
    if qkv.numel() != B * S * 3 * H * 64:
        raise ValueError(f"attention_fwd: qkv has {qkv.numel()} elements, expected B*S*3*H*64 = {B * S * 3 * H * 64}")
    out = torch.empty((B * S, H * 64), dtype=torch.float32, device=qkv.device)
    lse = torch.empty((B, H, S), dtype=torch.float32, device=qkv.device)
    _lib.check(lib.dclip_attention_fwd(qkv.data_ptr(), out.data_ptr(), lse.data_ptr(), B, S, H, int(causal),
                                       _stream()), "attention_fwd")
    return out, lse


def attention_bwd(qkv, out, dout, lse, B: int, S: int, H: int, causal: bool):
    lib = _lib.load()
    _f32(qkv, "qkv"), _f32(out, "out"), _f32(dout, "dout"), _f32(lse, "lse")
    if qkv.numel() != B * S * 3 * H * 64 or out.numel() != B * S * H * 64 or dout.numel() != out.numel() \
            or lse.numel() != B * H * S:
        raise ValueError("attention_bwd: shape mismatch")
    dqkv = torch.empty_like(qkv)
    nbytes = int(lib.dclip_attention_bwd_workspace(B, S, H, int(causal)))
    ws = torch.empty((nbytes + 3) // 4, dtype=torch.float32, device=qkv.device)
    _lib.check(lib.dclip_attention_bwd_ws(qkv.data_ptr(), out.data_ptr(), dout.data_ptr(), lse.data_ptr(),
                                          dqkv.data_ptr(), ws.data_ptr(), nbytes, B, S, H, int(causal), _stream()),
               "attention_bwd")
    return dqkv


def attention_cls_fwd(qkv: torch.Tensor, B: int, S: int, H: int):
    lib = _lib.load()
    _f32(qkv, "qkv")
    if qkv.numel() != B * S * 3 * H * 64:
        raise ValueError("attention_cls_fwd: qkv size")
    out = torch.empty((B, H * 64), dtype=torch.float32, device=qkv.device)
    lse = torch.empty((B, H), dtype=torch.float32, device=qkv.device)
    _lib.check(lib.dclip_attention_cls_fwd(qkv.data_ptr(), out.data_ptr(), lse.data_ptr(), B, S, H, _stream()),
               "attention_cls_fwd")
    return out, lse


def attention_row_fwd(qkv: torch.Tensor, rows: torch.Tensor, B: int, S: int, H: int):
    lib = _lib.load()
    _f32(qkv, "qkv"), _idx(rows, B)
    if qkv.numel() != B * S * 3 * H * 64:
        raise ValueError("attention_row_fwd: qkv size")
    out = torch.empty((B, H * 64), dtype=torch.float32, device=qkv.device)
    lse = torch.empty((B, H), dtype=torch.float32, device=qkv.device)
    _lib.check(lib.dclip_attention_row_fwd(qkv.data_ptr(), rows.data_ptr(), out.data_ptr(), lse.data_ptr(), B, S, H,
                                           _stream()), "attention_row_fwd")
    return out


def attention_cls_bwd(qkv, out, dout, lse, B: int, S: int, H: int):
# ... 973 lines not shown
        extra = {"wt": tcopies, "dst_t": torch.tensor([by_dst[r[1]] for r in mats], dtype=torch.int64).to(dev)}
    return {**extra, "table": table, "nrefs": len(blob), "tiles": t0, "wrefs": len(mats), "wtiles": wtiles, "w": copies, "L": len(layers),
            "D": layers[0]["ln1_w"].numel(),
            "stats": torch.zeros((len(layers), len(SPLIT16_STATS)), dtype=torch.int32, device=dev),
            "plan": torch.zeros((len(layers), nplan), dtype=torch.float32, device=dev)}


def split16_refresh(tab) -> None:
    lib = _lib.load()
    st = _stream()
    _lib.check(lib.dclip_split16_stats(tab["table"].data_ptr(), tab["nrefs"], tab["tiles"], tab["stats"].data_ptr(), st),
               "split16_stats")
    _lib.check(lib.dclip_split16_plan(tab["stats"].data_ptr(), tab["plan"].data_ptr(), tab["L"], tab["D"], st), "split16_plan")
    if "dst_t" in tab:
        _lib.check(lib.dclip_split16_weights_t(tab["table"].data_ptr(), tab["wrefs"], tab["wtiles"], tab["plan"].data_ptr(),
                                               tab["dst_t"].data_ptr(), st), "split16_weights_t")
    else:
        _lib.check(lib.dclip_split16_weights(tab["table"].data_ptr(), tab["wrefs"], tab["wtiles"], tab["plan"].data_ptr(), st),
                   "split16_weights")


def split_f16x3_rows(x: torch.Tensor):
    lib = _lib.load()
    if x.dtype != torch.float32 or not x.is_cuda or x.dim() != 2 or x.stride(1) != 1:
        raise ValueError("split_f16x3_rows: x must be a 2-D fp32 device tensor with unit column stride")
    rows, cols = x.shape
    y = torch.empty((rows, 3 * cols), dtype=torch.float16, device=x.device)
    ra = torch.empty((rows,), dtype=torch.float32, device=x.device)
    _lib.check(lib.dclip_split_f32_f16x3_rows(x.data_ptr(), y.data_ptr(), ra.data_ptr(), rows, cols, x.stride(0) if rows > 1 else cols,
                                              _stream()), "split_f32_f16x3_rows")
    return y, ra


def gemm_f16_rows_dev(a: torch.Tensor, w: torch.Tensor, alpha_ptr: int, row_alpha: torch.Tensor,
                      dgelu_h: Optional[torch.Tensor] = None) -> torch.Tensor:
    lib = _lib.load()
    _f16(a, "a"), _f16(w, "w")
    M, lda = a.shape
    N, ldw = w.shape
    K = min(lda, ldw)
    if _f32(row_alpha, "row_alpha").numel() != M:
        raise ValueError("gemm_f16_rows_dev: row_alpha size")
    if dgelu_h is not None and tuple(_f32(dgelu_h, "dgelu_h").shape) != (M, N):
        raise ValueError("gemm_f16_rows_dev: dgelu_h shape")
    out = torch.empty((M, N), dtype=torch.float32, device=a.device)
    _lib.check(lib.dclip_gemm_f16_scaled_rows_dev(a.data_ptr(), w.data_ptr(), out.data_ptr(), _ptr(dgelu_h), M, N, K, lda, ldw, N,
                                                  EPI_DGELU if dgelu_h is not None else 0, alpha_ptr, row_alpha.data_ptr(),
                                                  _stream()), "gemm_f16_scaled_rows_dev")
    return out


def split_f16x3_rows_colstats(x: torch.Tensor, db: Optional[torch.Tensor] = None):
    lib = _lib.load()
    if x.dtype != torch.float32 or not x.is_cuda or x.dim() != 2 or x.stride(1) != 1:
        raise ValueError("split_f16x3_rows_colstats: x must be a 2-D fp32 device tensor with unit column stride")
    rows, cols = x.shape
    if db is not None and (_f32(db, "db").numel() != cols):
        raise ValueError("split_f16x3_rows_colstats: db size")
    dev = x.device
    y = torch.empty((rows, 3 * cols), dtype=torch.float16, device=dev)
    ra = torch.empty((rows,), dtype=torch.float32, device=dev)
    yc = torch.empty((rows, 2 * cols), dtype=torch.float16, device=dev)
    ce = torch.empty((cols,), dtype=torch.int32, device=dev)
    ca = torch.empty((cols,), dtype=torch.float32, device=dev)
    nbytes = lib.dclip_split_f32_f16x3_rows_colstats_workspace(rows, cols)
    ws = _ws.get(nbytes, dev)
    _lib.check(lib.dclip_split_f32_f16x3_rows_colstats(x.data_ptr(), y.data_ptr(), ra.data_ptr(), yc.data_ptr(), ce.data_ptr(),
                                                       ca.data_ptr(), _ptr(db), rows, cols, x.stride(0) if rows > 1 else cols,
                                                       _ptr(ws), nbytes, _stream()), "split_f32_f16x3_rows_colstats")
    return y, ra, yc, ce, ca


def gemm_f16_wgrad_tokmajor_seg3_plan(M: int, N: int, tokens: int) -> int:
    return int(_lib.load().dclip_gemm_f16_wgrad_tokmajor_seg3_plan(M, N, tokens))


def gemm_f16_wgrad_tokmajor_seg3(dy: torch.Tensor, x: torch.Tensor, M: int, N: int, col_alpha: torch.Tensor, act_scale_ptr: int,
                                 a_seg=None, w_seg=None, splits: Optional[int] = None,
                                 out: Optional[torch.Tensor] = None) -> Optional[torch.Tensor]:
    lib = _lib.load()
    _f16(dy, "dy"), _f16(x, "x")
    if dy.dim() != 2 or x.dim() != 2 or dy.shape[0] != x.shape[0]:
        raise ValueError("gemm_f16_wgrad_tokmajor_seg3: dy / x are [tokens, ld] with the same token count")
    tokens = dy.shape[0]
    a_seg = (0, M, 0) if a_seg is None else tuple(int(v) for v in a_seg)
    w_seg = (0, 0, N) if w_seg is None else tuple(int(v) for v in w_seg)
    if splits is None:
        splits = lib.dclip_gemm_f16_wgrad_tokmajor_seg3_plan(M, N, tokens)
        if splits == 0:
            return None
    if _f32(col_alpha, "col_alpha").numel() != M:
        raise ValueError("gemm_f16_wgrad_tokmajor_seg3: col_alpha size")
    out = _out_f32(out, (M, N), dy.device, "gemm_f16_wgrad_tokmajor_seg3")
    nbytes = lib.dclip_gemm_f16_splitk_workspace(M, N, 3 * splits)
    ws = _ws.get(nbytes, dy.device)
    _lib.check(lib.dclip_gemm_f16_wgrad_tokmajor_seg3(dy.data_ptr(), x.data_ptr(), out.data_ptr(), M, N, tokens, dy.shape[1], x.shape[1],
                                                      N, a_seg[0], a_seg[1], a_seg[2], w_seg[0], w_seg[1], w_seg[2],
                                                      col_alpha.data_ptr(), act_scale_ptr, splits, _ptr(ws), nbytes, _stream()),
               "gemm_f16_wgrad_tokmajor_seg3")
    return out


# ... 467 lines not shown
```

include/dclip_hip.h:

```cpp
#ifndef DCLIP_HIP_H
#define DCLIP_HIP_H

#include <stddef.h>
#include <stdint.h>

#ifdef __cplusplus
extern "C" {
#endif

#define DCLIP_ABI_VERSION 1

enum {
  DCLIP_OK = 0,
  DCLIP_EINVAL = -1,
  DCLIP_EWORKSPACE = -2,
  DCLIP_ELAUNCH = -3
};

int dclip_abi_version(void);
const char* dclip_last_error(void);
const char* dclip_last_launch(void);
const char* dclip_first_launch(void);

#define DCLIP_A_KMAJOR 1
// ... 201 lines not shown
                          int lda, int ldw, int ldc, int epilogue, int out_f16, float alpha, void* stream);
int dclip_gemm_f16_scaled_split(const void* A, const void* W, void* C, const float* bias, int M, int N, int K, int lda, int ldw,
                                int ldc, int epilogue, float alpha, float out_scale, void* stream);

int dclip_split_f32_f16x3_dev(const float* x, void* y, int rows, int cols, int ldx, int ldy, const float* scale, int order,
                              void* stream);
int dclip_layernorm_fwd_f16x3_dev(const float* x, const float* gamma, const float* beta, void* y, float* y32, float* mean,
                                  float* rstd, int rows, int D, float eps, const float* scale, void* stream);
int dclip_gemm_f16_scaled_dev(const void* A, const void* W, void* C, const float* bias, const float* residual, int M, int N, int K,
                              int lda, int ldw, int ldc, int epilogue, int out_f16, const float* alpha, void* stream);
int dclip_gemm_f16_scaled_split_dev(const void* A, const void* W, void* C, const float* bias, float* h32, float* g32, int M, int N,
                                    int K, int lda, int ldw, int ldc, int epilogue, const float* alpha, const float* out_scale,
                                    void* stream);
int dclip_split16_record_bytes(void);
int dclip_split16_plan_floats(void);
int dclip_split16_tile_rows(void);
int dclip_split16_stats(const void* refs, int nrefs, int tiles, void* stats, void* stream);
int dclip_split16_plan(void* stats, float* plan, int nlayers, int D, void* stream);
int dclip_split16_weights(const void* refs, int nrefs, int tiles, const float* plan, void* stream);

int dclip_split_f32_f16x3_rows(const float* x, void* y, float* row_alpha, int rows, int cols, int ldx, void* stream);
int dclip_split16_weights_t(const void* refs, int nrefs, int tiles, const float* plan, const void* dst_t, void* stream);
int dclip_gemm_f16_scaled_rows_dev(const void* A, const void* W, float* C, const float* aux32, int M, int N, int K, int lda, int ldw,
                                   int ldc, int epilogue, const float* alpha, const float* row_alpha, void* stream);

size_t dclip_split_f32_f16x3_rows_colstats_workspace(int rows, int cols);
int dclip_split_f32_f16x3_rows_colstats(const float* x, void* y, float* row_alpha, void* yc, int* col_exp, float* col_alpha, float* db,
                                        int rows, int cols, int ldx, void* workspace, size_t workspace_bytes, void* stream);
int dclip_gemm_f16_wgrad_tokmajor_seg3_plan(int M, int N, int tokens);
int dclip_gemm_f16_wgrad_tokmajor_seg3(const void* dY, const void* X, float* C, int M, int N, int tokens, int lddy, int ldx, int ldc,
                                       int a_seg0, int a_seg1, int a_seg2, int w_seg0, int w_seg1, int w_seg2, const float* col_alpha,
                                       const float* act_scale, int splits, void* workspace, size_t workspace_bytes, void* stream);

int dclip_gemm_f16_ex(const void* A, const void* W, void* C, const float* bias, const float* residual, void* aux, int M,
                      int N, int K, int lda, int ldw, int ldc, int epilogue, int out_f16, void* stream);
int dclip_gemm_f16_wgrad_tokmajor_plan(int M, int N, int K);
int dclip_gemm_f16_wgrad_tokmajor(const void* dY, const void* X, float* C, int M, int N, int K, int lddy, int ldx, int ldc,
                                  int splits, void* workspace, size_t workspace_bytes, void* stream);
int dclip_gemm_f16_splitk_plan(int M, int N, int K);
size_t dclip_gemm_f16_splitk_workspace(int M, int N, int splits);
int dclip_gemm_f16_splitk(const void* A, const void* W, float* C, int M, int N, int K, int lda, int ldw, int ldc, int splits,
                          void* workspace, size_t workspace_bytes, void* stream);
int dclip_cast_f32_f16_ieee(const float* x, void* y, int rows, int cols, int ldx, int ldy, void* stream);
int dclip_layernorm_fwd_f16_stats(const float* x, const float* gamma, const float* beta, void* y, float* mean, float* rstd,
                                  int rows, int D, float eps, void* stream);
int dclip_layernorm_bwd_ex_f16(const float* dy, const float* x, const float* gamma, const float* mean, const float* rstd,
                               const float* dresidual, float* dx, void* dx_f16, float* dgamma, float* dbeta, float* dx_colsum,
                               int rows, int D, int accumulate_param_grads, void* workspace, size_t workspace_bytes,
                               void* stream);
int dclip_transpose_to_f16(const void* x, int x_is_f16, void* yT, void* y_copy, int rows, int cols, int ldx, int ldyT,
                           int ldy, void* stream);
int dclip_rowsum_f16(const void* x, float* out, int R, int n, int ld, void* stream);
int dclip_colsum_f16(const void* X, float* out, int M, int N, int ldx, int accumulate, void* workspace,
                     size_t workspace_bytes, void* stream);
int dclip_mt_weights_f16(const void* refs, int ntensors, int total_tiles, void* stream);
int dclip_attention_fwd_f16_lse(const void* qkv, void* out, float* lse, int B, int S, int H, int causal, void* stream);
int dclip_attention_bwd_f16(const void* qkv, const void* out, const void* dout, const float* lse, void* dqkv, int B, int S,
                            int H, int causal, void* stream);
int dclip_clip_coef_scaled(const float* partial, int n, float max_norm, const float* scale, float* out, void* stream);
int dclip_mt_adamw_f32_skip(const void* refs, int ntensors, int total_chunks, float lr, float one_minus_beta1,
                            float one_minus_beta2, float eps, float weight_decay, const float* coef3, void* stream);
int dclip_amp_update_scale(float* scale, int* growth_tracker, const float* found_inf, float growth_factor,
                           float backoff_factor, int growth_interval, void* stream);

int dclip_axpby(const float* x, float* y, float a, float b, size_t n, void* stream);
int dclip_fill(float* y, float v, size_t n, void* stream);
// ... 6 lines not shown
```

Baseline: 7126.

## Fuse column max/sum statistics into backward producer kernels

```diff
diff --git a/dclip_amd/_lib.py b/dclip_amd/_lib.py
--- a/dclip_amd/_lib.py
+++ b/dclip_amd/_lib.py
@@ -141,6 +141,13 @@
     "dclip_gemm_f16_scaled_rows_dev": (I, [P, P, P, P, I, I, I, I, I, I, I, P, P, P]),
     "dclip_split_f32_f16x3_rows_colstats_workspace": (Z, [I, I]),
     "dclip_split_f32_f16x3_rows_colstats": (I, [P, P, P, P, P, P, P, I, I, I, P, Z, P]),
+    "dclip_split_f32_f16x3_rows_cols_stats": (I, [P, P, P, P, P, P, P, P, P, I, I, I, I, P]),
+    "dclip_gemm_f16_scaled_rows_stats_plan": (I, [I, I, I]),
+    "dclip_gemm_f16_scaled_rows_stats_dev": (I, [P, P, P, P, I, I, I, I, I, I, I, P, P, P, P, P]),
+    "dclip_attention_bwd_stats_plan": (I, [I, I, I]),
+    "dclip_attention_bwd_stats": (I, [P, P, P, P, P, P, P, I, I, I, I, P]),
+    "dclip_layernorm_bwd_stats_plan": (I, [I, I]),
+    "dclip_layernorm_bwd_stats": (I, [P, P, P, P, P, P, P, P, P, P, P, I, I, I, P, Z, P]),
     "dclip_gemm_f16_wgrad_tokmajor_seg3_plan": (I, [I, I, I]),
     "dclip_gemm_f16_wgrad_tokmajor_seg3": (I, [P, P, P, I, I, I, I, I, I, I, I, I, I, I, I, P, P, I, P, Z, P]),
     "dclip_gemm_f16_ex": (I, [P, P, P, P, P, P, I, I, I, I, I, I, I, I, P]),
diff --git a/dclip_amd/csrc/attention.hip b/dclip_amd/csrc/attention.hip
--- a/dclip_amd/csrc/attention.hip
+++ b/dclip_amd/csrc/attention.hip
@@ -567,11 +567,12 @@
   }
 }
 
-template <bool CAUSAL, bool IO16 = false>
-__global__ void __launch_bounds__(256, 3) attn_bwd_lean_kernel(AttnArgs a, const float* __restrict__ out,
-                                                               const float* __restrict__ dout, const float* __restrict__ lse,
-                                                               float* __restrict__ dq_out, float* __restrict__ dk_out,
-                                                               float* __restrict__ dv_out, int ldd) {
+template <bool CAUSAL, bool IO16, bool STATS>
+__device__ __forceinline__ void attn_bwd_lean_body(const AttnArgs& a, const float* __restrict__ out, const float* __restrict__ dout,
+                                                   const float* __restrict__ lse, float* __restrict__ dq_out,
+                                                   float* __restrict__ dk_out, float* __restrict__ dv_out, int ldd,
+                                                   unsigned* __restrict__ pmax, float* __restrict__ psum) {
+  static_assert(!STATS || !IO16, "the statistics form is fp32");
   __shared__ __attribute__((aligned(16))) float lds[3 * TS * HD + 2 * TS];
   float* Qs = lds;
   float* dOs = lds + TS * HD;
@@ -652,6 +653,7 @@
   }
   __syncthreads();
   const int kts = (S + 15) / 16;
+  f32x4 sk[STATS ? 4 : 1], sv[STATS ? 4 : 1];
   {
     f32x4 dk[4], dv[4];
     zero4(dk);
@@ -704,6 +706,10 @@
           *reinterpret_cast<f32x4*>(dv_out + o + 16 * dt) = dv[dt];
         }
       }
+    }
+    if constexpr (STATS) {
+#pragma unroll
+      for (int dt = 0; dt < 4; ++dt) sk[dt] = dk[dt], sv[dt] = dv[dt];
     }
   }
   __syncthreads();
@@ -738,7 +744,53 @@
         for (int dt = 0; dt < 4; ++dt) *reinterpret_cast<f32x4*>(o + 16 * dt) = dq[dt];
       }
     }
-  }
+    if constexpr (STATS) {
+      __syncthreads();
+      if (own < S) {
+#pragma unroll
+        for (int dt = 0; dt < 4; ++dt) {
+          const int o = tile_off(own, 16 * dt + 4 * qd);
+          *reinterpret_cast<f32x4*>(lds + o) = dq[dt];
+          *reinterpret_cast<f32x4*>(lds + TS * HD + o) = sk[dt];
+          *reinterpret_cast<f32x4*>(lds + 2 * TS * HD + o) = sv[dt];
+        }
+      }
+      __syncthreads();
+      const int c = threadIdx.x;
+      if (c < 3 * HD) {
+        const int mt = c >> 6, cc = c & 63;
+        const float* t = lds + mt * TS * HD;
+        unsigned m = 0u;
+        float s = 0.f;
+        for (int r = 0; r < S; ++r) {
+          const float v = t[tile_off(r, cc)];
+          const unsigned u = __builtin_bit_cast(unsigned, v) & 0x7fffffffu;
+          m = m > u ? m : u;
+          s += v;
+        }
+        const size_t o = (size_t)b * 3 * D + (size_t)mt * D + h * HD + cc;
+        pmax[o] = m;
+        psum[o] = s;
+      }
+    }
+  }
+}
+
+template <bool CAUSAL, bool IO16 = false>
+__global__ void __launch_bounds__(256, 3) attn_bwd_lean_kernel(AttnArgs a, const float* __restrict__ out,
+                                                               const float* __restrict__ dout, const float* __restrict__ lse,
+                                                               float* __restrict__ dq_out, float* __restrict__ dk_out,
+                                                               float* __restrict__ dv_out, int ldd) {
+  attn_bwd_lean_body<CAUSAL, IO16, false>(a, out, dout, lse, dq_out, dk_out, dv_out, ldd, nullptr, nullptr);
+}
+
+template <bool CAUSAL>
+__global__ void __launch_bounds__(256, 3) attn_bwd_lean_stats_kernel(AttnArgs a, const float* __restrict__ out,
+                                                                     const float* __restrict__ dout, const float* __restrict__ lse,
+                                                                     float* __restrict__ dq_out, float* __restrict__ dk_out,
+                                                                     float* __restrict__ dv_out, int ldd,
+                                                                     unsigned* __restrict__ pmax, float* __restrict__ psum) {
+  attn_bwd_lean_body<CAUSAL, false, true>(a, out, dout, lse, dq_out, dk_out, dv_out, ldd, pmax, psum);
 }
 
 
@@ -1323,6 +1375,26 @@
   return launch_bwd(a, out, dout, lse, dqkv, 3 * D, dqkv + D, dqkv + 2 * D, 3 * D, delta, B, causal, (hipStream_t)stream);
 }
 
+DCLIP_API int dclip_attention_bwd_stats_plan(int B, int S, int H) { return B > 0 && H > 0 && S > 1 && S <= TS ? B : 0; }
+
+DCLIP_API int dclip_attention_bwd_stats(const float* qkv, const float* out, const float* dout, const float* lse, float* dqkv,
+                                        void* pmax, float* psum, int B, int S, int H, int causal, void* stream) {
+  DCLIP_REQUIRE(qkv && out && dout && lse && dqkv && pmax && psum, "attention_bwd_stats: null pointer");
+  DCLIP_REQUIRE(dclip_attention_bwd_stats_plan(B, S, H) > 0, "attention_bwd_stats: no such form for B=%d S=%d H=%d", B, S, H);
+  DCLIP_REQUIRE(((uintptr_t)pmax | (uintptr_t)psum) % 4 == 0, "attention_bwd_stats: alignment");
+  const int D = H * HD;
+  AttnArgs a{qkv, qkv + D, qkv + 2 * D, 3 * D, 3 * D, S, S, H, nullptr};
+  hipStream_t st = (hipStream_t)stream;
+  if (causal)
+    hipLaunchKernelGGL((attn_bwd_lean_stats_kernel<true>), dim3(B * H), dim3(256), 0, st, a, out, dout, lse, dqkv, dqkv + D,
+                       dqkv + 2 * D, 3 * D, (unsigned*)pmax, psum);
+  else
+    hipLaunchKernelGGL((attn_bwd_lean_stats_kernel<false>), dim3(B * H), dim3(256), 0, st, a, out, dout, lse, dqkv, dqkv + D,
+                       dqkv + 2 * D, 3 * D, (unsigned*)pmax, psum);
+  DCLIP_CHECK_LAUNCH("attention_bwd.lean.stats");
+  return DCLIP_OK;
+}
+
 DCLIP_API size_t dclip_attention_bwd_workspace(int B, int S, int H, int causal) {
   size_t n = (size_t)B * H * S;
   n = (n + 63) / 64 * 64;
diff --git a/dclip_amd/csrc/gemm_bf16.hip b/dclip_amd/csrc/gemm_bf16.hip
--- a/dclip_amd/csrc/gemm_bf16.hip
+++ b/dclip_amd/csrc/gemm_bf16.hip
@@ -34,6 +34,8 @@
   const float* aux32 = nullptr;
   int seg_splits = 0;
   int a_seg[3] = {0, 0, 0}, w_seg[3] = {0, 0, 0};
+  unsigned* pmax = nullptr;
+  float* psum = nullptr;
 };
 
 __device__ __forceinline__ void store_rows4(const GemmBf16Params& p, f32x4 v, int row, size_t off) {
@@ -317,7 +319,7 @@
     __builtin_amdgcn_sched_barrier(0);    \
   } while (0)
 
-template <class T, int KIND, bool OUT16, bool DEV = false, bool ROWS = false>
+template <class T, int KIND, bool OUT16, bool DEV = false, bool ROWS = false, bool STATS = false>
 __device__ __forceinline__ void pp_epilogue(const GemmBf16Params& p, const f32x4 (&acc)[8][4], float* ct, int m0, int n0,
                                             int tid, int wr, int wc, int quad, int l15) {
   constexpr int BN = 256;
@@ -327,6 +329,13 @@
   f32x4 bias4 = {0.f, 0.f, 0.f, 0.f};
   if (p.epilogue & DCLIP_EPI_BIAS) bias4 = *reinterpret_cast<const f32x4*>(p.bias + colc);
   const float alpha_d = DEV ? *p.alpha_p : 0.f;
+  static_assert(!STATS || ROWS, "the statistics form is the row-scaled one");
+  unsigned smx[STATS ? 4 : 1];
+  float ssm[STATS ? 4 : 1];
+  if constexpr (STATS) {
+#pragma unroll
+    for (int e = 0; e < 4; ++e) smx[e] = 0u, ssm[e] = 0.f;
+  }
 #pragma unroll
   for (int hm = 0; hm < 2; ++hm) {
     const int rbase = m0 + hm * 128 + lr0;
@@ -369,6 +378,15 @@
           for (int e = 0; e < 4; ++e) v[e] *= quick_gelu_grad_f(side[q][e]);
         }
         if (ok) *reinterpret_cast<f32x4*>(reinterpret_cast<float*>(p.C) + off) = v;
+        if constexpr (STATS) if (ok) {
+#pragma unroll
+          for (int e = 0; e < 4; ++e) {
+            const float ve = v[e];
+            const unsigned u = __builtin_bit_cast(unsigned, ve) & 0x7fffffffu;
+            smx[e] = smx[e] > u ? smx[e] : u;
+            ssm[e] += ve;
+          }
+        }
         continue;
       }
       if (KIND == 1) {
@@ -407,6 +425,29 @@
     }
   }
   PP_STAMP(8);
+  if constexpr (STATS) {
+    asm volatile("s_waitcnt lgkmcnt(0)" ::: "memory");
+    PP_BARRIER();
+    unsigned* cu = reinterpret_cast<unsigned*>(ct);
+    float* cs = ct + 8 * BN;
+    *reinterpret_cast<u32x4*>(cu + lr0 * BN + lc) = u32x4{smx[0], smx[1], smx[2], smx[3]};
+    *reinterpret_cast<f32x4*>(cs + lr0 * BN + lc) = f32x4{ssm[0], ssm[1], ssm[2], ssm[3]};
+    asm volatile("s_waitcnt lgkmcnt(0)" ::: "memory");
+    PP_BARRIER();
+    if (tid < BN && n0 + tid < p.N) {
+      unsigned m = cu[tid];
+      float sm = cs[tid];
+#pragma unroll
+      for (int w = 1; w < 8; ++w) {
+        const unsigned mw = cu[w * BN + tid];
+        m = m > mw ? m : mw;
+        sm += cs[w * BN + tid];
+      }
+      const size_t o = (size_t)(m0 / 256) * p.N + n0 + tid;
+      p.pmax[o] = m;
+      p.psum[o] = sm;
+    }
+  }
 #ifdef DCLIP_GEMM_STAMPS
   asm volatile("s_waitcnt vmcnt(0)" ::: "memory");
 #endif
@@ -473,9 +514,10 @@
   PP_STAMP_RT(6);
 }
 
-template <class T, bool TOK, bool DEV = false, bool ROWS = false, bool SEG = false>
+template <class T, bool TOK, bool DEV = false, bool ROWS = false, bool SEG = false, bool STATS = false>
 __global__ void __launch_bounds__(512) gemm_bf16_pp_kernel(GemmBf16Params p) {
   static_assert(!SEG || (TOK && !DEV && !ROWS), "the segmented form is token-major, split-K, fp32 slabs");
+  static_assert(!STATS || (ROWS && !TOK), "the statistics form is the row-scaled dgrad");
   typedef typename T::x8 V8;
   constexpr int BM = 256, BN = 256, ROW = BKH;
   constexpr int BUF = (BM + BN) * ROW;
@@ -697,8 +739,8 @@
     for (int i = 0; i < 8; ++i)
 #pragma unroll
       for (int j = 0; j < 4; ++j) acc[i][j] = (acc[i][j] * alpha_r) * ra[i];
-    if (kind == 2) pp_epilogue<T, 2, false, true, true>(p, acc, ct, m0, n0, tid, wr, wc, quad, l15);
-    else pp_epilogue<T, 0, false, true, true>(p, acc, ct, m0, n0, tid, wr, wc, quad, l15);
+    if (kind == 2) pp_epilogue<T, 2, false, true, true, STATS>(p, acc, ct, m0, n0, tid, wr, wc, quad, l15);
+    else pp_epilogue<T, 0, false, true, true, STATS>(p, acc, ct, m0, n0, tid, wr, wc, quad, l15);
     return;
   }
   if (!DEV && p.slab) {
@@ -1038,6 +1080,11 @@
   p.tiles_m = cdiv(p.M, 256);
   p.tiles_n = cdiv(p.N, 256);
   if constexpr (std::is_same<T, F16T>::value && !TOK) {
+    if (p.row_alpha && p.pmax) {
+      hipLaunchKernelGGL((gemm_bf16_pp_kernel<T, false, true, true, false, true>), dim3(p.tiles_m * p.tiles_n, splits), dim3(512), 0,
+                         st, p);
+      return DCLIP_OK;
+    }
     if (p.row_alpha) {
       hipLaunchKernelGGL((gemm_bf16_pp_kernel<T, false, true, true>), dim3(p.tiles_m * p.tiles_n, splits), dim3(512), 0, st, p);
       return DCLIP_OK;
@@ -1171,11 +1218,16 @@
   float* g32;
   const float* row_alpha = nullptr;
   const float* aux32 = nullptr;
+  unsigned* pmax = nullptr;
+  float* psum = nullptr;
 };
 inline void set_dev(GemmBf16Params& p, const DevScales* d) {
   if (d) p.alpha_p = d->alpha_p, p.out_scale_p = d->out_scale_p, p.h32 = d->h32, p.g32 = d->g32, p.row_alpha = d->row_alpha,
-         p.aux32 = d->aux32;
-}
+         p.aux32 = d->aux32, p.pmax = d->pmax, p.psum = d->psum;
+}
+
+inline int pp_big_min() { return getenv("DCLIP_BF16_BIG_MIN") ? atoi(getenv("DCLIP_BF16_BIG_MIN")) : 128; }
+inline bool takes_pp(int M, int N, int K) { return K % BKH == 0 && (long)cdiv(M, 256) * cdiv(N, 256) >= pp_big_min(); }
 
 template <class T>
 constexpr bool kTrain16 = std::is_same<T, F16IeeeT>::value;
@@ -1199,8 +1251,7 @@
   DCLIP_REQUIRE(!(epilogue & DCLIP_EPI_BIAS) || bias, "%s: BIAS without bias", name);
   DCLIP_REQUIRE(!(epilogue & DCLIP_EPI_RESIDUAL) || (residual && !out_bf16), "%s: RESIDUAL needs an fp32 output", name);
   hipStream_t st = (hipStream_t)stream;
-  const int big_min = getenv("DCLIP_BF16_BIG_MIN") ? atoi(getenv("DCLIP_BF16_BIG_MIN")) : 128;
-  if (K % BKH == 0 && (long)cdiv(M, 256) * cdiv(N, 256) >= big_min) {
+  if (takes_pp(M, N, K)) {
     GemmBf16Params pb{(const __bf16*)A, (const __bf16*)W, C, bias, residual, M, N, K, lda, ldw, ldc, epilogue, out_bf16, 0, 0,
                       (unsigned short*)aux, 0, nullptr, alpha, out_scale};
     set_dev(pb, dev);
@@ -1297,6 +1348,30 @@
   dev.aux32 = (epilogue & DCLIP_EPI_DGELU) ? aux32 : nullptr;
   return gemm16<F16T>("gemm_f16_scaled_rows_dev", A, W, C, nullptr, nullptr, nullptr, M, N, K, lda, ldw, ldc, epilogue, 0, stream, 1.f,
                       0.f, &dev);
+}
+
+DCLIP_API int dclip_gemm_f16_scaled_rows_stats_plan(int M, int N, int K) {
+  return M > 0 && N > 0 && K > 0 && takes_pp(M, N, K) ? cdiv(M, 256) : 0;
+}
+
+DCLIP_API int dclip_gemm_f16_scaled_rows_stats_dev(const void* A, const void* W, float* C, const float* aux32, int M, int N, int K,
+                                                   int lda, int ldw, int ldc, int epilogue, const float* alpha, const float* row_alpha,
+                                                   void* pmax, float* psum, void* stream) {
+  DCLIP_REQUIRE(alpha && row_alpha && ((uintptr_t)alpha | (uintptr_t)row_alpha) % 4 == 0,
+                "gemm_f16_scaled_rows_stats_dev: alpha / row_alpha must be device pointers");
+  DCLIP_REQUIRE(pmax && psum && ((uintptr_t)pmax | (uintptr_t)psum) % 4 == 0, "gemm_f16_scaled_rows_stats_dev: pmax / psum");
+  DCLIP_REQUIRE(epilogue == 0 || epilogue == DCLIP_EPI_DGELU, "gemm_f16_scaled_rows_stats_dev: the epilogue is none or DGELU");
+  DCLIP_REQUIRE(!(epilogue & DCLIP_EPI_DGELU) || (aux32 && (uintptr_t)aux32 % 16 == 0),
+                "gemm_f16_scaled_rows_stats_dev: DGELU needs a 16-byte aligned fp32 aux32");
+  DCLIP_REQUIRE(dclip_gemm_f16_scaled_rows_stats_plan(M, N, K) > 0,
+                "gemm_f16_scaled_rows_stats_dev: M=%d N=%d K=%d takes a register-staged kernel, which has no statistics form", M, N, K);
+  DevScales dev{alpha, nullptr, nullptr, nullptr};
+  dev.row_alpha = row_alpha;
+  dev.aux32 = (epilogue & DCLIP_EPI_DGELU) ? aux32 : nullptr;
+  dev.pmax = (unsigned*)pmax;
+  dev.psum = psum;
+  return gemm16<F16T>("gemm_f16_scaled_rows_dev.stats", A, W, C, nullptr, nullptr, nullptr, M, N, K, lda, ldw, ldc, epilogue, 0, stream,
+                      1.f, 0.f, &dev);
 }
 
 DCLIP_API int dclip_gemm_f16_ex(const void* A, const void* W, void* C, const float* bias, const float* residual, void* aux,
diff --git a/dclip_amd/csrc/layernorm.hip b/dclip_amd/csrc/layernorm.hip
--- a/dclip_amd/csrc/layernorm.hip
+++ b/dclip_amd/csrc/layernorm.hip
@@ -50,16 +50,18 @@
   }
 }
 
-template <class T, int NC, bool EXACT>
-__global__ void __launch_bounds__(256) ln_bwd_kernel(const float* __restrict__ dy, const float* __restrict__ x,
-                                                     const float* __restrict__ gamma, const float* __restrict__ mean,
-                                                     const float* __restrict__ rstd, const float* __restrict__ dres,
-                                                     float* __restrict__ dx, float* __restrict__ partial, int rows,
-                                                     int D, unsigned short* __restrict__ dx16, int NS) {
+template <class T, int NC, bool EXACT, bool STATS>
+__device__ __forceinline__ void ln_bwd_body(const float* __restrict__ dy, const float* __restrict__ x,
+                                            const float* __restrict__ gamma, const float* __restrict__ mean,
+                                            const float* __restrict__ rstd, const float* __restrict__ dres,
+                                            float* __restrict__ dx, float* __restrict__ partial, int rows, int D,
+                                            unsigned short* __restrict__ dx16, int NS, unsigned* __restrict__ pmax,
+                                            float* __restrict__ psum) {
   extern __shared__ __attribute__((aligned(16))) float red[];
   const int lane = threadIdx.x & 63, wave = threadIdx.x >> 6;
   const int d4 = D >> 2;
   f32x4 g[NC], dg[NC], db[NC], dsum[NC];
+  unsigned dmx[STATS ? NC : 1][4];
 #pragma unroll
   for (int c = 0; c < NC; ++c) {
     int i = lane + 64 * c;
@@ -67,6 +69,7 @@
     dg[c] = f32x4{0.f, 0.f, 0.f, 0.f};
     db[c] = f32x4{0.f, 0.f, 0.f, 0.f};
     dsum[c] = f32x4{0.f, 0.f, 0.f, 0.f};
+    if constexpr (STATS) dmx[c][0] = dmx[c][1] = dmx[c][2] = dmx[c][3] = 0u;
   }
   const float invD = 1.0f / (float)D;
   const bool has_res = dres != nullptr;
@@ -110,6 +113,14 @@
         if (has_res) o += rv[c];
         dxr[i] = o;
         if (NS == 3) dsum[c] += o;
+        if constexpr (STATS) {
+#pragma unroll
+          for (int e = 0; e < 4; ++e) {
+            const float oe = o[e];
+            const unsigned u = __builtin_bit_cast(unsigned, oe) & 0x7fffffffu;
+            dmx[c][e] = dmx[c][e] > u ? dmx[c][e] : u;
+          }
+        }
         if (dx16) {
           typedef unsigned short u16x4_t __attribute__((ext_vector_type(4)));
           u16x4_t b;
@@ -119,6 +130,33 @@
         }
       }
     }
+  }
+  if constexpr (STATS) {
+    typedef unsigned int u32x4_t __attribute__((ext_vector_type(4)));
+#pragma unroll
+    for (int c = 0; c < NC; ++c) {
+      int i = lane + 64 * c;
+      if (EXACT || i < d4) {
+        reinterpret_cast<f32x4*>(red + (wave * 4 + 0) * D)[i] = dg[c];
+        reinterpret_cast<f32x4*>(red + (wave * 4 + 1) * D)[i] = db[c];
+        reinterpret_cast<f32x4*>(red + (wave * 4 + 2) * D)[i] = dsum[c];
+        reinterpret_cast<u32x4_t*>(red + (wave * 4 + 3) * D)[i] = u32x4_t{dmx[c][0], dmx[c][1], dmx[c][2], dmx[c][3]};
+      }
+    }
+    __syncthreads();
+    const int W = 4 * D;
+    for (int i = threadIdx.x; i < W; i += 256) {
+      if (i < 3 * D) {
+        float s = red[i] + red[W + i] + red[2 * W + i] + red[3 * W + i];
+        if (i >= 2 * D) psum[(size_t)blockIdx.x * D + (i - 2 * D)] = s;
+        else if (partial) partial[(size_t)blockIdx.x * 2 * D + i] = s;
+      } else {
+        const unsigned* ru = reinterpret_cast<const unsigned*>(red);
+        const unsigned m01 = ru[i] > ru[W + i] ? ru[i] : ru[W + i], m23 = ru[2 * W + i] > ru[3 * W + i] ? ru[2 * W + i] : ru[3 * W + i];
+        pmax[(size_t)blockIdx.x * D + (i - 3 * D)] = m01 > m23 ? m01 : m23;
+      }
+    }
+    return;
   }
   if (partial) {
 #pragma unroll
@@ -137,6 +175,104 @@
       partial[(size_t)blockIdx.x * W + i] = s;
     }
   }
+}
+
+template <class T, int NC, bool EXACT>
+__global__ void __launch_bounds__(256) ln_bwd_kernel(const float* __restrict__ dy, const float* __restrict__ x,
+                                                     const float* __restrict__ gamma, const float* __restrict__ mean,
+                                                     const float* __restrict__ rstd, const float* __restrict__ dres,
+                                                     float* __restrict__ dx, float* __restrict__ partial, int rows,
+                                                     int D, unsigned short* __restrict__ dx16, int NS) {
+  extern __shared__ __attribute__((aligned(16))) float red[];
+  const int lane = threadIdx.x & 63, wave = threadIdx.x >> 6;
+  const int d4 = D >> 2;
+  f32x4 g[NC], dg[NC], db[NC], dsum[NC];
+#pragma unroll
+  for (int c = 0; c < NC; ++c) {
+    int i = lane + 64 * c;
+    g[c] = (EXACT || i < d4) ? reinterpret_cast<const f32x4*>(gamma)[i] : f32x4{0.f, 0.f, 0.f, 0.f};
+    dg[c] = f32x4{0.f, 0.f, 0.f, 0.f};
+    db[c] = f32x4{0.f, 0.f, 0.f, 0.f};
+    dsum[c] = f32x4{0.f, 0.f, 0.f, 0.f};
+  }
+  const float invD = 1.0f / (float)D;
+  const bool has_res = dres != nullptr;
+  for (int row = blockIdx.x * 4 + wave; row < rows; row += gridDim.x * 4) {
+    const f32x4* xr = reinterpret_cast<const f32x4*>(x + (size_t)row * D);
+    const f32x4* dyr = reinterpret_cast<const f32x4*>(dy + (size_t)row * D);
+    const f32x4* rr = reinterpret_cast<const f32x4*>((has_res ? dres : dy) + (size_t)row * D);
+    const float mu = mean[row], rs = rstd[row];
+    f32x4 xh[NC], dyh[NC], rv[NC];
+#pragma unroll
+    for (int c = 0; c < NC; ++c) {
+      const int i = lane + 64 * c, ic = (EXACT || i < d4) ? i : 0;
+      dyh[c] = dyr[ic];
+      xh[c] = xr[ic];
+      rv[c] = rr[ic];
+    }
+    float s1 = 0.f, s2 = 0.f;
+#pragma unroll
+    for (int c = 0; c < NC; ++c) {
+      if (EXACT || lane + 64 * c < d4) {
+        const f32x4 dyv = dyh[c];
+        xh[c] = (xh[c] - mu) * rs;
+        dg[c] += dyv * xh[c];
+        db[c] += dyv;
+        dyh[c] = dyv * g[c];
+        f32x4 t = dyh[c] * xh[c];
+        s1 += (t[0] + t[1]) + (t[2] + t[3]);
+        s2 += (dyh[c][0] + dyh[c][1]) + (dyh[c][2] + dyh[c][3]);
+      } else {
+        xh[c] = f32x4{0.f, 0.f, 0.f, 0.f};
+        dyh[c] = f32x4{0.f, 0.f, 0.f, 0.f};
+      }
+    }
+    const float c1 = wave_sum(s1) * invD, c2 = wave_sum(s2) * invD;
+    f32x4* dxr = reinterpret_cast<f32x4*>(dx + (size_t)row * D);
+#pragma unroll
+    for (int c = 0; c < NC; ++c) {
+      const int i = lane + 64 * c;
+      if (EXACT || i < d4) {
+        f32x4 o = (dyh[c] - c2 - xh[c] * c1) * rs;
+        if (has_res) o += rv[c];
+        dxr[i] = o;
+        if (NS == 3) dsum[c] += o;
+        if (dx16) {
+          typedef unsigned short u16x4_t __attribute__((ext_vector_type(4)));
+          u16x4_t b;
+#pragma unroll
+          for (int e = 0; e < 4; ++e) b[e] = T::bits(o[e]);
+          *reinterpret_cast<u16x4_t*>(dx16 + (size_t)row * D + i * 4) = b;
+        }
+      }
+    }
+  }
+  if (partial) {
+#pragma unroll
+    for (int c = 0; c < NC; ++c) {
+      int i = lane + 64 * c;
+      if (EXACT || i < d4) {
+        reinterpret_cast<f32x4*>(red + (wave * NS + 0) * D)[i] = dg[c];
+        reinterpret_cast<f32x4*>(red + (wave * NS + 1) * D)[i] = db[c];
+        if (NS == 3) reinterpret_cast<f32x4*>(red + (wave * NS + 2) * D)[i] = dsum[c];
+      }
+    }
+    __syncthreads();
+    const int W = NS * D;
+    for (int i = threadIdx.x; i < W; i += 256) {
+      float s = red[i] + red[W + i] + red[2 * W + i] + red[3 * W + i];
+      partial[(size_t)blockIdx.x * W + i] = s;
+    }
+  }
+}
+
+template <class T, int NC, bool EXACT>
+__global__ void __launch_bounds__(256) ln_bwd_stats_kernel(const float* __restrict__ dy, const float* __restrict__ x,
+                                                           const float* __restrict__ gamma, const float* __restrict__ mean,
+                                                           const float* __restrict__ rstd, const float* __restrict__ dres,
+                                                           float* __restrict__ dx, float* __restrict__ partial, int rows, int D,
+                                                           unsigned* __restrict__ pmax, float* __restrict__ psum) {
+  ln_bwd_body<T, NC, EXACT, true>(dy, x, gamma, mean, rstd, dres, dx, partial, rows, D, nullptr, 3, pmax, psum);
 }
 
 constexpr int RP_COLS = 16, RP_GROUPS = 64;
@@ -357,6 +493,52 @@
                                    rows, D, accumulate_param_grads, workspace, workspace_bytes, stream);
 }
 
+DCLIP_API int dclip_layernorm_bwd_stats_plan(int rows, int D) {
+  if (rows <= 0 || D <= 0 || D % 4 || D > 1024) return 0;
+  return ln_bwd_blocks(rows);
+}
+
+DCLIP_API int dclip_layernorm_bwd_stats(const float* dy, const float* x, const float* gamma, const float* mean, const float* rstd,
+                                        const float* dresidual, float* dx, float* dgamma, float* dbeta, void* pmax, float* psum,
+                                        int rows, int D, int accumulate_param_grads, void* workspace, size_t workspace_bytes,
+                                        void* stream) {
+  DCLIP_REQUIRE(dy && x && gamma && mean && rstd && dx && pmax && psum, "layernorm_bwd_stats: null pointer");
+  DCLIP_REQUIRE(dclip_layernorm_bwd_stats_plan(rows, D) > 0, "layernorm_bwd_stats: no such form for rows=%d D=%d", rows, D);
+  DCLIP_REQUIRE(((uintptr_t)pmax | (uintptr_t)psum) % 4 == 0, "layernorm_bwd_stats: alignment");
+  const bool want_params = dgamma || dbeta;
+  const int blocks = ln_bwd_blocks(rows);
+  if (want_params && (!workspace || workspace_bytes < dclip_layernorm_bwd_workspace(rows, D))) {
+    dclip_set_error("layernorm_bwd_stats: workspace too small (%zu < %zu)", workspace_bytes, dclip_layernorm_bwd_workspace(rows, D));
+    return DCLIP_EWORKSPACE;
+  }
+  float* partial = want_params ? (float*)workspace : nullptr;
+  hipStream_t st = (hipStream_t)stream;
+  const size_t lds = (size_t)4 * 4 * D * sizeof(float);
+  const int nc = cdiv(D / 4, 64);
+  const char* variant;
+#define LN_BWDS(NC, EX)                                                                                                          \
+  do {                                                                                                                           \
+    hipLaunchKernelGGL((ln_bwd_stats_kernel<Bf16T, NC, EX>), dim3(blocks), dim3(256), lds, st, dy, x, gamma, mean, rstd, dresidual, \
+                       dx, partial, rows, D, (unsigned*)pmax, psum);                                                             \
+    variant = (EX) ? ".nc" #NC ".exact" : ".nc" #NC;                                                                             \
+  } while (0)
+  if (D == 512) LN_BWDS(2, true);
+  else if (D == 768) LN_BWDS(3, true);
+  else if (D == 1024) LN_BWDS(4, true);
+  else if (nc <= 1) LN_BWDS(1, false);
+  else if (nc == 2) LN_BWDS(2, false);
+  else if (nc == 3) LN_BWDS(3, false);
+  else LN_BWDS(4, false);
+#undef LN_BWDS
+  DCLIP_CHECK_LAUNCH_V("layernorm_bwd_stats", variant);
+  if (want_params) {
+    hipLaunchKernelGGL(reduce_partials_kernel, dim3(cdiv(2 * D, RP_COLS)), dim3(1024), 0, st, partial, dgamma, dbeta, blocks, D, D,
+                       accumulate_param_grads, (float*)nullptr, 0);
+    DCLIP_CHECK_LAUNCH_V("layernorm_bwd_stats", variant);
+  }
+  return DCLIP_OK;
+}
+
 DCLIP_API size_t dclip_colsum_f32_workspace(int M, int N) { return (size_t)colsum_splits(M) * N * sizeof(float); }
 
 DCLIP_API int dclip_colsum_f32(const float* X, float* out, int M, int N, int ldx, int accumulate, void* workspace,
diff --git a/dclip_amd/csrc/split16.hip b/dclip_amd/csrc/split16.hip
--- a/dclip_amd/csrc/split16.hip
+++ b/dclip_amd/csrc/split16.hip
@@ -283,6 +283,82 @@
     unsigned short* yr = yc + r * 2 * cols + c;
     *reinterpret_cast<u16x8*>(yr) = hi;
     *reinterpret_cast<u16x8*>(yr + cols) = lo;
+  }
+}
+
+__device__ __forceinline__ void split_cols_store8(unsigned short* yr, int cols, const f32x4& a, const f32x4& b,
+                                                  const int* __restrict__ ce) {
+  const i32x4s ea = *reinterpret_cast<const i32x4s*>(ce), eb = *reinterpret_cast<const i32x4s*>(ce + 4);
+  u16x8 hi, lo;
+#pragma unroll
+  for (int e = 0; e < 4; ++e) {
+    unsigned short h0, l0, h1, l1;
+    split1(a[e] * pow2f(ea[e]), h0, l0);
+    split1(b[e] * pow2f(eb[e]), h1, l1);
+    hi[e] = h0, lo[e] = l0, hi[4 + e] = h1, lo[4 + e] = l1;
+  }
+  *reinterpret_cast<u16x8*>(yr) = hi;
+  *reinterpret_cast<u16x8*>(yr + cols) = lo;
+}
+
+__device__ __forceinline__ void split_store8_nt(unsigned short* yr, int cols, const f32x4& a, const f32x4& b, float scale) {
+  u16x8 hi, lo;
+#pragma unroll
+  for (int e = 0; e < 4; ++e) {
+    unsigned short h0, l0, h1, l1;
+    split1(a[e] * scale, h0, l0);
+    split1(b[e] * scale, h1, l1);
+    hi[e] = h0, lo[e] = l0, hi[4 + e] = h1, lo[4 + e] = l1;
+  }
+  __builtin_nontemporal_store(hi, reinterpret_cast<u16x8*>(yr));
+  __builtin_nontemporal_store(lo, reinterpret_cast<u16x8*>(yr + cols));
+  __builtin_nontemporal_store(hi, reinterpret_cast<u16x8*>(yr + 2 * cols));
+}
+
+template <int NC>
+__global__ void __launch_bounds__(256) split_rows_cols_f16_kernel(const float* __restrict__ x, unsigned short* __restrict__ y,
+                                                                  float* __restrict__ row_alpha, const int* __restrict__ col_exp,
+                                                                  unsigned short* __restrict__ yc, int rows, int cols, int ldx) {
+  const int lane = threadIdx.x & 63;
+  const int row = blockIdx.x * 4 + (threadIdx.x >> 6);
+  if (row >= rows) return;
+  const int c8 = cols >> 3;
+  const float* xr = x + (size_t)row * ldx;
+  unsigned short* yr = y + (size_t)row * 3 * cols;
+  unsigned short* ycr = yc + (size_t)row * 2 * cols;
+  unsigned m = 0u;
+  if (NC > 0) {
+    f32x4 a[NC > 0 ? NC : 1], b[NC > 0 ? NC : 1];
+#pragma unroll
+    for (int c = 0; c < NC; ++c) {
+      const int i = lane + 64 * c, ic = i < c8 ? i : 0;
+      a[c] = *reinterpret_cast<const f32x4*>(xr + ic * 8);
+      b[c] = *reinterpret_cast<const f32x4*>(xr + ic * 8 + 4);
+    }
+#pragma unroll
+    for (int c = 0; c < NC; ++c) m = absmax8(m, a[c], b[c]);
+    const int e = row_exp(wave_umax_bits(m));
+    const float scale = pow2f(e);
+    if (lane == 0) row_alpha[row] = pow2f(-e);
+#pragma unroll
+    for (int c = 0; c < NC; ++c) {
+      const int i = lane + 64 * c;
+      if (i < c8) {
+        split_store8_nt(yr + i * 8, cols, a[c], b[c], scale);
+        split_cols_store8(ycr + i * 8, cols, a[c], b[c], col_exp + i * 8);
+      }
+    }
+  } else {
+    for (int i = lane; i < c8; i += 64)
+      m = absmax8(m, *reinterpret_cast<const f32x4*>(xr + i * 8), *reinterpret_cast<const f32x4*>(xr + i * 8 + 4));
+    const int e = row_exp(wave_umax_bits(m));
+    const float scale = pow2f(e);
+    if (lane == 0) row_alpha[row] = pow2f(-e);
+    for (int i = lane; i < c8; i += 64) {
+      const f32x4 a = *reinterpret_cast<const f32x4*>(xr + i * 8), b = *reinterpret_cast<const f32x4*>(xr + i * 8 + 4);
+      split_store8_nt(yr + i * 8, cols, a, b, scale);
+      split_cols_store8(ycr + i * 8, cols, a, b, col_exp + i * 8);
+    }
   }
 }
 
@@ -618,6 +694,30 @@
   return DCLIP_OK;
 }
 
+int split_rows_cols_launch(const float* x, void* y, float* row_alpha, const int* col_exp, void* yc, int rows, int cols, int ldx,
+                           void* stream) {
+  dim3 grid(cdiv(rows, 4)), block(256);
+  hipStream_t st = (hipStream_t)stream;
+  unsigned short *yy = (unsigned short*)y, *yyc = (unsigned short*)yc;
+  const int nc = cdiv(cols / 8, 64);
+  const char* variant;
+#define SPLITROWSCOLS(NC)                                                                                                          \
+  do {                                                                                                                             \
+    hipLaunchKernelGGL((split_rows_cols_f16_kernel<NC>), grid, block, 0, st, x, yy, row_alpha, col_exp, yyc, rows, cols, ldx);     \
+    variant = (NC) ? ".regs.nc" #NC : ".cached";                                                                                   \
+  } while (0)
+  if (nc <= 1) SPLITROWSCOLS(1);
+  else if (nc == 2) SPLITROWSCOLS(2);
+  else if (nc == 3) SPLITROWSCOLS(3);
+  else if (nc == 4) SPLITROWSCOLS(4);
+  else if (nc == 5) SPLITROWSCOLS(5);
+  else if (nc == 6) SPLITROWSCOLS(6);
+  else SPLITROWSCOLS(0);
+#undef SPLITROWSCOLS
+  DCLIP_CHECK_LAUNCH_V("split_f32_f16x3_rows_cols_stats", variant);
+  return DCLIP_OK;
+}
+
 int ln_launch(const char* name, const float* x, const float* gamma, const float* beta, void* y, int rows, int D, float eps,
               float scale, const float* scale_p, float* y32, float* mean, float* rstd, void* stream) {
   dim3 grid(cdiv(rows, 4)), block(256);
@@ -713,6 +813,25 @@
   return DCLIP_OK;
 }
 
+DCLIP_API int dclip_split_f32_f16x3_rows_cols_stats(const float* x, void* y, float* row_alpha, void* yc, int* col_exp, float* col_alpha,
+                                                    float* db, const void* pmax, const float* psum, int P, int rows, int cols, int ldx,
+                                                    void* stream) {
+  dclip_note_first_launch("", "");
+  DCLIP_REQUIRE(x && y && row_alpha && yc && col_exp && col_alpha && pmax && psum && P > 0 && rows > 0 && cols > 0,
+                "split_f32_f16x3_rows_cols_stats: bad arguments");
+  DCLIP_REQUIRE(cols % 8 == 0, "split_f32_f16x3_rows_cols_stats: cols=%d must be a multiple of 8", cols);
+  DCLIP_REQUIRE(ldx >= cols && ldx % 4 == 0, "split_f32_f16x3_rows_cols_stats: ldx must be a multiple of 4 and >= cols");
+  DCLIP_REQUIRE(((uintptr_t)x | (uintptr_t)y | (uintptr_t)yc | (uintptr_t)col_exp) % 16 == 0 &&
+                    ((uintptr_t)row_alpha | (uintptr_t)col_alpha | (uintptr_t)db | (uintptr_t)pmax | (uintptr_t)psum) % 4 == 0,
+                "split_f32_f16x3_rows_cols_stats: alignment");
+  hipStream_t st = (hipStream_t)stream;
+  hipLaunchKernelGGL(colstats_finish_kernel, dim3(cdiv(cols, FIN_COLS)), dim3(256), 0, st, (const unsigned*)pmax, psum, col_exp, col_alpha,
+                     db, P, cols);
+  DCLIP_CHECK_LAUNCH_V("split_f32_f16x3_rows_cols_stats", ".finish");
+  dclip_note_first_launch("split_f32_f16x3_rows_cols_stats", ".finish");
+  return split_rows_cols_launch(x, y, row_alpha, (const int*)col_exp, yc, rows, cols, ldx, stream);
+}
+
 DCLIP_API int dclip_layernorm_fwd_f16x3(const float* x, const float* gamma, const float* beta, void* y, int rows, int D,
                                         float eps, float scale, void* stream) {
   DCLIP_REQUIRE(x && gamma && beta && y, "layernorm_fwd_f16x3: null pointer");
diff --git a/dclip_amd/engine.py b/dclip_amd/engine.py
--- a/dclip_amd/engine.py
+++ b/dclip_amd/engine.py
@@ -104,11 +104,14 @@
 def linear_param_grads(dy, x, need_w: bool, need_b: bool, gr: Dict[str, torch.Tensor], wkey: str, bkey: str, alloc=None,
                        sp: Optional[Split16Layer] = None, act: Optional[str] = None, x3: Optional[torch.Tensor] = None):
     dev = dy.device
-    if (need_w and sp is not None and x3 is not None and _VSPLIT16_WGRAD and dy.dim() == 2 and dy.stride(1) == 1 and
-            ops.gemm_f16_wgrad_tokmajor_seg3_plan(dy.shape[1], x.shape[1], dy.shape[0]) > 0):
+    if dy.dim() == 2 and dy.stride(1) == 1 and _split_wgrad_taken(need_w, sp, x3, dy.shape[1], x.shape[1], dy.shape[0]):
         M, N = dy.shape[1], x.shape[1]
         db = _galloc(alloc, bkey, (M,), dev) if need_b else None
-        dy3, row_alpha, yc, _, col_alpha = ops.split_f16x3_rows_colstats(dy, db=db)
+        st = getattr(dy, "dystats", None) if _VSPLIT16_DYSTATS else None
+        if st is not None:
+            dy3, row_alpha, yc, _, col_alpha = ops.split_f16x3_rows_cols_stats(dy, st, db=db)
+        else:
+            dy3, row_alpha, yc, _, col_alpha = ops.split_f16x3_rows_colstats(dy, db=db)
         if need_b:
             gr[bkey] = db
         gr[wkey] = ops.gemm_f16_wgrad_tokmajor_seg3(yc, x3, M, N, col_alpha, sp.act(act), out=_galloc(alloc, wkey, (M, N), dev))
@@ -123,47 +126,78 @@
     return None
 
 
-def _ln_bwd(dy, x, gamma, mean, rstd, dresidual, want: bool, gr, wkey: str, bkey: str, alloc):
+def _split_wgrad_taken(need_w: bool, sp: Optional[Split16Layer], x3, out_f: int, in_f: int, tokens: int) -> bool:
+    return bool(need_w and sp is not None and x3 is not None and _VSPLIT16_WGRAD and
+                ops.gemm_f16_wgrad_tokmajor_seg3_plan(out_f, in_f, tokens) > 0)
+
+
+def _dystats_regime(tokens: int, D: int, I: int) -> bool:
+    return bool(_VSPLIT16_DYSTATS and ops.gemm_f16_rows_stats_plan(tokens, I, 3 * D) > 0)
+
+
+def _with_stats(want: bool, P: int, cols: int, dev):
+    return ops.ColStats(P, cols, dev) if want and _VSPLIT16_DYSTATS and P > 0 else None
+
+
+def _ln_bwd(dy, x, gamma, mean, rstd, dresidual, want: bool, gr, wkey: str, bkey: str, alloc, dx_stats: bool = False):
+    D = x.shape[-1]
+    st = _with_stats(dx_stats, ops.layernorm_bwd_stats_plan(x.numel() // D, D) if dx_stats else 0, D, dy.device)
     if want:
         dg = _galloc(alloc, wkey, tuple(gamma.shape), dy.device)
         db = _galloc(alloc, bkey, tuple(gamma.shape), dy.device)
-        dx, dg, db = ops.layernorm_bwd(dy, x, gamma, mean, rstd, dresidual=dresidual, dgamma=dg, dbeta=db, accumulate=False)
+        dx, dg, db = ops.layernorm_bwd(dy, x, gamma, mean, rstd, dresidual=dresidual, dgamma=dg, dbeta=db, accumulate=False, stats=st)
         gr[wkey], gr[bkey] = dg, db
-        return dx
-    dx, _, _ = ops.layernorm_bwd(dy, x, gamma, mean, rstd, dresidual=dresidual, need_param_grads=False)
+    else:
+        dx, _, _ = ops.layernorm_bwd(dy, x, gamma, mean, rstd, dresidual=dresidual, need_param_grads=False, stats=st)
+    if st is not None:
+        dx.dystats = st
     return dx
 
 
-def _dgrad(dy, w, sp: Optional[Split16Layer], name: str, aux=None, rows=None):
+def _dgrad(dy, w, sp: Optional[Split16Layer], name: str, aux=None, rows=None, out_stats: bool = False):
     if sp is None:
         if aux is None:
             return ops.gemm(dy, w, ops.LAYOUT_NN)
         return ops.gemm(dy, w, ops.LAYOUT_NN, aux=aux, epilogue=ops.EPI_DGELU)
     dy3, row_alpha = rows if rows is not None else ops.split_f16x3_rows(dy)
-    return ops.gemm_f16_rows_dev(dy3, sp.wt[name], sp.walpha(name), row_alpha, dgelu_h=aux)
+    wt = sp.wt[name]
+    st = _with_stats(out_stats, ops.gemm_f16_rows_stats_plan(dy3.shape[0], wt.shape[0], min(dy3.shape[1], wt.shape[1]))
+                     if out_stats else 0, wt.shape[0], dy3.device)
+    dx = ops.gemm_f16_rows_dev(dy3, wt, sp.walpha(name), row_alpha, dgelu_h=aux, stats=st)
+    if st is not None:
+        dx.dystats = st
+    return dx
 
 
 def layer_bwd(dx2, p: LayerParams, saved, B: int, S: int, H: int, causal: bool, need: Dict[str, bool], alloc=None,
-              sp: Optional[Split16Layer] = None):
+              sp: Optional[Split16Layer] = None, dx_stats: bool = False, dystats: bool = False):
     x, m1, r1, ln1, qkv, attn, lse, x1, m2, r2, ln2, h, g = saved[:13]
     s3 = saved[13] if len(saved) > 13 and sp is not None else {}
     gr: Dict[str, torch.Tensor] = {}
+    T, D, I = x.shape[0], x.shape[1], p.fc1_w.shape[0]
     rows = linear_param_grads(dx2, g, bool(need.get("fc2_w")), bool(need.get("fc2_b")), gr, "fc2_w", "fc2_b", alloc, sp, "g", s3.get("g"))
-    dh = _dgrad(dx2, p.fc2_w, sp, "fc2", aux=h, rows=rows)
+    dh = _dgrad(dx2, p.fc2_w, sp, "fc2", aux=h, rows=rows,
+                out_stats=dystats and _split_wgrad_taken(bool(need.get("fc1_w")), sp, s3.get("ln2"), I, D, T))
     rows = linear_param_grads(dh, ln2, bool(need.get("fc1_w")), bool(need.get("fc1_b")), gr, "fc1_w", "fc1_b", alloc, sp, "ln2",
                               s3.get("ln2"))
     dln2 = _dgrad(dh, p.fc1_w, sp, "fc1", rows=rows)
     del dh
-    dx1 = _ln_bwd(dln2, x1, p.ln2_w, m2, r2, dx2, bool(need.get("ln2_w") or need.get("ln2_b")), gr, "ln2_w", "ln2_b", alloc)
+    dx1 = _ln_bwd(dln2, x1, p.ln2_w, m2, r2, dx2, bool(need.get("ln2_w") or need.get("ln2_b")), gr, "ln2_w", "ln2_b", alloc,
+                  dx_stats=dystats and _split_wgrad_taken(bool(need.get("out_w")), sp, s3.get("ctx"), D, D, T))
     rows = linear_param_grads(dx1, attn, bool(need.get("out_w")), bool(need.get("out_b")), gr, "out_w", "out_b", alloc, sp, "ctx",
                               s3.get("ctx"))
     dattn = _dgrad(dx1, p.out_w, sp, "out", rows=rows)
-    dqkv = ops.attention_bwd(qkv, attn, dattn, lse, B, S, H, causal)
+    qkv_stats = dystats and _split_wgrad_taken(bool(need.get("qkv_w")), sp, s3.get("ln1"), 3 * D, D, T)
+    st = _with_stats(qkv_stats, ops.attention_bwd_stats_plan(B, S, H) if qkv_stats else 0, 3 * D, dattn.device)
+    dqkv = ops.attention_bwd(qkv, attn, dattn, lse, B, S, H, causal, stats=st)
+    if st is not None:
+        dqkv.dystats = st
     rows = linear_param_grads(dqkv, ln1, bool(need.get("qkv_w")), bool(need.get("qkv_b")), gr, "qkv_w", "qkv_b", alloc, sp, "ln1",
                               s3.get("ln1"))
     dln1 = _dgrad(dqkv, p.qkv_w, sp, "qkv", rows=rows)
     del dqkv, rows
-    dx = _ln_bwd(dln1, x, p.ln1_w, m1, r1, dx1, bool(need.get("ln1_w") or need.get("ln1_b")), gr, "ln1_w", "ln1_b", alloc)
+    dx = _ln_bwd(dln1, x, p.ln1_w, m1, r1, dx1, bool(need.get("ln1_w") or need.get("ln1_b")), gr, "ln1_w", "ln1_b", alloc,
+                 dx_stats=dx_stats)
     return dx, gr
 
 
@@ -187,7 +221,7 @@
 
 
 def last_layer_bwd_cls(dx2, p: LayerParams, saved, B: int, S: int, H: int, need: Dict[str, bool], alloc=None,
-                       sp: Optional[Split16Layer] = None):
+                       sp: Optional[Split16Layer] = None, dx_stats: bool = False):
     x, m1, r1, ln1, qkv, attn, lse, x1, m2, r2, ln2, h, g = saved[:13]
     s3 = saved[13] if len(saved) > 13 and sp is not None else {}
     D = x.shape[1]
@@ -205,7 +239,8 @@
     dln1 = _dgrad(dqkv, p.qkv_w, sp, "qkv", rows=rows)
     del dqkv, rows
     dres = ops.scatter_rows(dx1, None, B, S, D)
-    dx = _ln_bwd(dln1, x, p.ln1_w, m1, r1, dres, bool(need.get("ln1_w") or need.get("ln1_b")), gr, "ln1_w", "ln1_b", alloc)
+    dx = _ln_bwd(dln1, x, p.ln1_w, m1, r1, dres, bool(need.get("ln1_w") or need.get("ln1_b")), gr, "ln1_w", "ln1_b", alloc,
+                 dx_stats=dx_stats)
     return dx, gr
 
 
@@ -331,14 +366,18 @@
         return [grads[n] for n in names]
     dx = None if pruned else ops.scatter_rows(dcls, None, B, S, D)
     plan = split16.layers if split16 is not None and _VSPLIT16_BWD and split16.fresh() else None
+    dystats = plan is not None and _dystats_regime(B * S, D, p.layers[0].fc1_w.shape[0])
     for i in range(n_layers - 1, max(lowest, 0) - 1, -1):
         lneed = {f: needd[f"layers.{i}.{f}"] for f in LayerParams.FIELDS}
         lalloc = None if alloc is None else (lambda f, shape, i=i: alloc(f"layers.{i}.{f}", shape))
         sp = plan[i] if plan is not None else None
+        below = dystats and i - 1 >= max(lowest, 0) and len(saved_layers[i - 1]) > 13
+        dxs = below and _split_wgrad_taken(bool(needd[f"layers.{i - 1}.fc2_w"]), plan[i - 1], saved_layers[i - 1][13].get("g"),
+                                           D, p.layers[i - 1].fc1_w.shape[0], B * S)
         if pruned and i == n_layers - 1:
-            dx, gr = last_layer_bwd_cls(dcls, p.layers[i], saved_layers[i], B, S, H, lneed, lalloc, sp)
+            dx, gr = last_layer_bwd_cls(dcls, p.layers[i], saved_layers[i], B, S, H, lneed, lalloc, sp, dxs)
         else:
-            dx, gr = layer_bwd(dx, p.layers[i], saved_layers[i], B, S, H, False, lneed, lalloc, sp)
+            dx, gr = layer_bwd(dx, p.layers[i], saved_layers[i], B, S, H, False, lneed, lalloc, sp, dxs, dystats)
         saved_layers[i] = None
         for f, t in gr.items():
             grads[f"layers.{i}.{f}"] = t
@@ -1106,6 +1145,7 @@
 _VSPLIT16_FC1_EPI = os.environ.get("DCLIP_VISION_SPLIT16_FC1_EPI", "1") != "0"
 _VSPLIT16_BWD = os.environ.get("DCLIP_VISION_SPLIT16_BWD", "1") != "0"
 _VSPLIT16_WGRAD = os.environ.get("DCLIP_VISION_SPLIT16_WGRAD", "1") != "0"
+_VSPLIT16_DYSTATS = os.environ.get("DCLIP_VISION_SPLIT16_DYSTATS", "1") != "0"
 
 
 def vision_split16_enabled() -> bool:
diff --git a/dclip_amd/ops.py b/dclip_amd/ops.py
--- a/dclip_amd/ops.py
+++ b/dclip_amd/ops.py
@@ -69,6 +69,28 @@
         global _ws
         _ws = self.prev
         return False
+
+
+class ColStats:
+    __slots__ = ("pmax", "psum", "P", "cols")
+
+    def __init__(self, P: int, cols: int, device):
+        ws = _stats_lanes.setdefault(id(_ws), _Workspace()).get(2 * P * cols * 4, device)
+        self.pmax = ws[:P * cols * 4].view(torch.int32).view(P, cols)
+        self.psum = ws[P * cols * 4:2 * P * cols * 4].view(torch.float32).view(P, cols)
+        self.P, self.cols = P, cols
+
+    @classmethod
+    def of(cls, pmax: torch.Tensor, psum: torch.Tensor) -> "ColStats":
+        if pmax.dtype != torch.int32 or psum.dtype != torch.float32 or pmax.shape != psum.shape or pmax.dim() != 2 or \
+                not (pmax.is_contiguous() and psum.is_contiguous() and pmax.is_cuda and psum.is_cuda):
+            raise ValueError("ColStats.of: pmax int32 / psum fp32, contiguous device tensors of one shape [P, cols]")
+        st = cls.__new__(cls)
+        st.pmax, st.psum, (st.P, st.cols) = pmax, psum, pmax.shape
+        return st
+
+
+_stats_lanes = {}
 
 
 
@@ -153,7 +175,7 @@
 
 def layernorm_bwd(dy, x, gamma, mean, rstd, *, dresidual=None, dgamma=None, dbeta=None, accumulate=False,
                   need_param_grads=True, want_bf16: bool = False, dx_colsum: Optional[torch.Tensor] = None,
-                  dtype16: torch.dtype = torch.bfloat16):
+                  dtype16: torch.dtype = torch.bfloat16, stats: Optional[ColStats] = None):
     lib = _lib.load()
     _f32(dy, "dy"), _f32(x, "x"), _f32(gamma, "gamma"), _f32(mean, "mean"), _f32(rstd, "rstd")
     D = x.shape[-1]
@@ -177,6 +199,14 @@
         raise ValueError("layernorm_bwd: dx_colsum size")
     nbytes = lib.dclip_layernorm_bwd_workspace(rows, D) if (need_param_grads or dx_colsum is not None) else 0
     ws = _ws.get(nbytes, x.device)
+    if stats is not None:
+        if want_bf16 or dx_colsum is not None or (stats.P, stats.cols) != (layernorm_bwd_stats_plan(rows, D), D) or stats.P == 0:
+            raise ValueError("layernorm_bwd: stats go with the plain fp32 call and layernorm_bwd_stats_plan's row count")
+        _lib.check(lib.dclip_layernorm_bwd_stats(dy.data_ptr(), x.data_ptr(), gamma.data_ptr(), mean.data_ptr(), rstd.data_ptr(),
+                                                 _ptr(dresidual), dx.data_ptr(), _ptr(dgamma), _ptr(dbeta), stats.pmax.data_ptr(),
+                                                 stats.psum.data_ptr(), rows, D, int(accumulate), _ptr(ws), nbytes, _stream()),
+                   "layernorm_bwd_stats")
+        return dx, dgamma, dbeta
     if not want_bf16 and dx_colsum is None:
         _lib.check(lib.dclip_layernorm_bwd(dy.data_ptr(), x.data_ptr(), gamma.data_ptr(), mean.data_ptr(),
                                            rstd.data_ptr(), _ptr(dresidual), dx.data_ptr(), _ptr(dgamma), _ptr(dbeta),
@@ -193,6 +223,10 @@
     return (dx, dgamma, dbeta, dx16) if want_bf16 else (dx, dgamma, dbeta)
 
 
+def layernorm_bwd_stats_plan(rows: int, D: int) -> int:
+    return int(_lib.load().dclip_layernorm_bwd_stats_plan(rows, D))
+
+
 
 def attention_fwd(qkv: torch.Tensor, B: int, S: int, H: int, causal: bool):
     lib = _lib.load()
@@ -206,13 +240,24 @@
     return out, lse
 
 
-def attention_bwd(qkv, out, dout, lse, B: int, S: int, H: int, causal: bool):
+def attention_bwd_stats_plan(B: int, S: int, H: int) -> int:
+    return int(_lib.load().dclip_attention_bwd_stats_plan(B, S, H))
+
+
+def attention_bwd(qkv, out, dout, lse, B: int, S: int, H: int, causal: bool, stats: Optional[ColStats] = None):
     lib = _lib.load()
     _f32(qkv, "qkv"), _f32(out, "out"), _f32(dout, "dout"), _f32(lse, "lse")
     if qkv.numel() != B * S * 3 * H * 64 or out.numel() != B * S * H * 64 or dout.numel() != out.numel() \
             or lse.numel() != B * H * S:
         raise ValueError("attention_bwd: shape mismatch")
     dqkv = torch.empty_like(qkv)
+    if stats is not None:
+        if (stats.P, stats.cols) != (attention_bwd_stats_plan(B, S, H), 3 * H * 64) or stats.P == 0:
+            raise ValueError("attention_bwd: stats must have attention_bwd_stats_plan's row count and 3 H 64 columns")
+        _lib.check(lib.dclip_attention_bwd_stats(qkv.data_ptr(), out.data_ptr(), dout.data_ptr(), lse.data_ptr(), dqkv.data_ptr(),
+                                                 stats.pmax.data_ptr(), stats.psum.data_ptr(), B, S, H, int(causal), _stream()),
+                   "attention_bwd_stats")
+        return dqkv
     nbytes = int(lib.dclip_attention_bwd_workspace(B, S, H, int(causal)))
     ws = torch.empty((nbytes + 3) // 4, dtype=torch.float32, device=qkv.device)
     _lib.check(lib.dclip_attention_bwd_ws(qkv.data_ptr(), out.data_ptr(), dout.data_ptr(), lse.data_ptr(),
@@ -1252,8 +1297,12 @@
     return y, ra
 
 
+def gemm_f16_rows_stats_plan(M: int, N: int, K: int) -> int:
+    return int(_lib.load().dclip_gemm_f16_scaled_rows_stats_plan(M, N, K))
+
+
 def gemm_f16_rows_dev(a: torch.Tensor, w: torch.Tensor, alpha_ptr: int, row_alpha: torch.Tensor,
-                      dgelu_h: Optional[torch.Tensor] = None) -> torch.Tensor:
+                      dgelu_h: Optional[torch.Tensor] = None, stats: Optional[ColStats] = None) -> torch.Tensor:
     lib = _lib.load()
     _f16(a, "a"), _f16(w, "w")
     M, lda = a.shape
@@ -1264,6 +1313,14 @@
     if dgelu_h is not None and tuple(_f32(dgelu_h, "dgelu_h").shape) != (M, N):
         raise ValueError("gemm_f16_rows_dev: dgelu_h shape")
     out = torch.empty((M, N), dtype=torch.float32, device=a.device)
+    if stats is not None:
+        if (stats.P, stats.cols) != (gemm_f16_rows_stats_plan(M, N, K), N) or stats.P == 0:
+            raise ValueError("gemm_f16_rows_dev: stats must have gemm_f16_rows_stats_plan's row count and N columns")
+        _lib.check(lib.dclip_gemm_f16_scaled_rows_stats_dev(a.data_ptr(), w.data_ptr(), out.data_ptr(), _ptr(dgelu_h), M, N, K, lda, ldw,
+                                                            N, EPI_DGELU if dgelu_h is not None else 0, alpha_ptr,
+                                                            row_alpha.data_ptr(), stats.pmax.data_ptr(), stats.psum.data_ptr(),
+                                                            _stream()), "gemm_f16_scaled_rows_stats_dev")
+        return out
     _lib.check(lib.dclip_gemm_f16_scaled_rows_dev(a.data_ptr(), w.data_ptr(), out.data_ptr(), _ptr(dgelu_h), M, N, K, lda, ldw, N,
                                                   EPI_DGELU if dgelu_h is not None else 0, alpha_ptr, row_alpha.data_ptr(),
                                                   _stream()), "gemm_f16_scaled_rows_dev")
@@ -1288,6 +1345,28 @@
     _lib.check(lib.dclip_split_f32_f16x3_rows_colstats(x.data_ptr(), y.data_ptr(), ra.data_ptr(), yc.data_ptr(), ce.data_ptr(),
                                                        ca.data_ptr(), _ptr(db), rows, cols, x.stride(0) if rows > 1 else cols,
                                                        _ptr(ws), nbytes, _stream()), "split_f32_f16x3_rows_colstats")
+    return y, ra, yc, ce, ca
+
+
+def split_f16x3_rows_cols_stats(x: torch.Tensor, stats: ColStats, db: Optional[torch.Tensor] = None):
+    lib = _lib.load()
+    if x.dtype != torch.float32 or not x.is_cuda or x.dim() != 2 or x.stride(1) != 1:
+        raise ValueError("split_f16x3_rows_cols_stats: x must be a 2-D fp32 device tensor with unit column stride")
+    rows, cols = x.shape
+    if stats.cols != cols or stats.P <= 0:
+        raise ValueError("split_f16x3_rows_cols_stats: stats columns")
+    if db is not None and (_f32(db, "db").numel() != cols):
+        raise ValueError("split_f16x3_rows_cols_stats: db size")
+    dev = x.device
+    y = torch.empty((rows, 3 * cols), dtype=torch.float16, device=dev)
+    ra = torch.empty((rows,), dtype=torch.float32, device=dev)
+    yc = torch.empty((rows, 2 * cols), dtype=torch.float16, device=dev)
+    ce = torch.empty((cols,), dtype=torch.int32, device=dev)
+    ca = torch.empty((cols,), dtype=torch.float32, device=dev)
+    _lib.check(lib.dclip_split_f32_f16x3_rows_cols_stats(x.data_ptr(), y.data_ptr(), ra.data_ptr(), yc.data_ptr(), ce.data_ptr(),
+                                                         ca.data_ptr(), _ptr(db), stats.pmax.data_ptr(), stats.psum.data_ptr(), stats.P,
+                                                         rows, cols, x.stride(0) if rows > 1 else cols, _stream()),
+               "split_f32_f16x3_rows_cols_stats")
     return y, ra, yc, ce, ca
 
 
diff --git a/include/dclip_hip.h b/include/dclip_hip.h
--- a/include/dclip_hip.h
+++ b/include/dclip_hip.h
@@ -257,6 +257,20 @@
                                        int a_seg0, int a_seg1, int a_seg2, int w_seg0, int w_seg1, int w_seg2, const float* col_alpha,
                                        const float* act_scale, int splits, void* workspace, size_t workspace_bytes, void* stream);
 
+int dclip_split_f32_f16x3_rows_cols_stats(const float* x, void* y, float* row_alpha, void* yc, int* col_exp, float* col_alpha, float* db,
+                                          const void* pmax, const float* psum, int P, int rows, int cols, int ldx, void* stream);
+int dclip_gemm_f16_scaled_rows_stats_plan(int M, int N, int K);
+int dclip_gemm_f16_scaled_rows_stats_dev(const void* A, const void* W, float* C, const float* aux32, int M, int N, int K, int lda,
+                                         int ldw, int ldc, int epilogue, const float* alpha, const float* row_alpha, void* pmax,
+                                         float* psum, void* stream);
+int dclip_attention_bwd_stats_plan(int B, int S, int H);
+int dclip_attention_bwd_stats(const float* qkv, const float* out, const float* dout, const float* lse, float* dqkv, void* pmax,
+                              float* psum, int B, int S, int H, int causal, void* stream);
+int dclip_layernorm_bwd_stats_plan(int rows, int D);
+int dclip_layernorm_bwd_stats(const float* dy, const float* x, const float* gamma, const float* mean, const float* rstd,
+                              const float* dresidual, float* dx, float* dgamma, float* dbeta, void* pmax, float* psum, int rows, int D,
+                              int accumulate_param_grads, void* workspace, size_t workspace_bytes, void* stream);
+
 int dclip_gemm_f16_ex(const void* A, const void* W, void* C, const float* bias, const float* residual, void* aux, int M,
                       int N, int K, int lda, int ldw, int ldc, int epilogue, int out_f16, void* stream);
 int dclip_gemm_f16_wgrad_tokmajor_plan(int M, int N, int K);
```

Result: faster. 7324 (median of 6 runs) (+2.8%).
